# FudanCVL/SynFMC

Measured on AMD Instinct MI355X. Metric: denoising steps/sec, 16x320x512 bf16 U-Net+CMC+OMC, higher is better.
Workload: dtype bf16; 1 GPU; 16x320x512 clip, CFG batch 2, full-width 3D U-Net (1.39B params, random init) + Camera Adapter (CMC) + Object Motion Control (OMC) features, DDIM step; configs/obj.yaml shapes; 1 clip per GPU; frames=16, height=320, width=512, hip_graph=True, fp8_temporal_attention=False, parallelism=dp1 (independent clips, no collective)

## Files before the change

### include/fmc_hip.h

```cpp
#ifndef FMC_HIP_H
#define FMC_HIP_H

#include <stdint.h>

#ifdef __cplusplus
extern "C" {
#endif

#define FMC_VERSION 100

enum { FMC_BF16 = 0, FMC_F32 = 1 };

enum {
    FMC_OK = 0,
    FMC_E_SHAPE = -1,
    FMC_E_DTYPE = -2,
    FMC_E_ALIGN = -3,
    FMC_E_LAUNCH = -4,
    FMC_E_NULL = -5
};

int fmc_version(void);
const char* fmc_last_error(void);

int64_t fmc_groupnorm_workspace_bytes(int N, int C, int G);
int fmc_groupnorm_silu_fwd(const void* x, void* y, const float* gamma, const float* beta, float* stats,
                           void* workspace, int N, int HW, int C, int G, float eps, int act, int dtype,
                           const void* x2, int C1, void* stream);
int fmc_groupnorm_silu_bwd(const void* dy, const void* x, void* dx, const float* gamma, const float* beta,
                           const float* stats, void* workspace, int N, int HW, int C, int G, int act,
                           int dtype, void* stream);

int fmc_layernorm_fwd(const void* x, void* y, const float* gamma, const float* beta, const float* pe,
                      int64_t M, int C, float eps, int pe_inner, int pe_frames, int dtype, void* stream);
int fmc_layernorm_add_fwd(const void* x, const void* addend, void* sum_out, void* y, const float* gamma, const float* beta,
                          const float* pe, int64_t M, int C, float eps, int pe_inner, int pe_frames, int dtype, void* stream);

int fmc_geglu_fwd(const void* x, void* y, int64_t M, int Cff, int dtype, void* stream);

int fmc_spatial_attn_fwd(const void* q, const void* k, const void* v, void* o, float* lse, int B, int H,
                         int Sq, int Skv, int D, int64_t q_batch_stride, int64_t q_row_stride,
                         int64_t kv_batch_stride, int64_t kv_row_stride, int64_t o_batch_stride,
                         int64_t o_row_stride, int kv_batch_div, float scale, int dtype, void* stream);

int fmc_temporal_attn_fwd(const void* q, const void* k, const void* v, void* o, int n_clips, int n_pix,
                          int F, int H, int D, int64_t clip_stride, int64_t frame_stride,
                          int64_t pix_stride, int64_t o_clip_stride, int64_t o_frame_stride,
                          int64_t o_pix_stride, float scale, int dtype, void* stream);

int fmc_plucker_fwd(const float* K, const float* c2w, void* out, int B, int F, int H, int W, int c2w_rows,
                    int layout, int dtype, void* stream);

int fmc_omc_rasterize_fwd(const float* poses, const float* masks, void* feat, float* mask_out, int BF,
                          int n_obj, int H, int W, int layout, int dtype, void* stream);

int fmc_gaussian_circle_mask_fwd(const float* circles, float* out, int N, int H, int W, void* stream);

int fmc_mask_modulate_fwd(const void* x, const float* mask_in, void* y, float* mask_out, int N, int h, int w,
                          int C, int Hin, int Win, int dtype, void* stream);

int fmc_feature_add_fwd(const void* h, const void* t, void* out, int64_t n_elems, int64_t skip_elems,
                        int dtype, void* stream);

int fmc_cfg_ddim_step(const void* eps_uc, const float* x, float* x_out, int64_t n, int has_uncond,
                      float guidance, float alpha_t, float alpha_prev, int dtype, void* stream);

int fmc_linear_bf16(const void* x, const void* w, const void* bias, const void* residual, void* out, int64_t M, int N,
                    int K, int64_t ldx, int64_t ldres, int64_t ldo, float alpha, int epilogue, int tile, int split_k,
                    void* workspace, int64_t workspace_bytes, const void* x2, int64_t ldx2, int k_split,
                    const void* residual2, void* stream);

int fmc_conv3x3_bf16(const void* x, const void* w, const void* bias, const void* temb, const void* residual, void* out,
                     int n_img, int H, int W, int Cin, int Cout, int64_t temb_row_stride, int temb_img_div,
                     int upsample2x, int tile, int split_k, void* workspace, int64_t workspace_bytes, void* stream);

int fmc_linear_bf16_gn(const void* x, const void* w, const void* bias, const void* residual, void* out, int64_t M, int N, int K,
                       int64_t ldx, int64_t ldres, int64_t ldo, float alpha, const void* residual2, float* gn_partials, int gn_hw,
                       int w_tilemajor, void* stream);
int fmc_linear_bf16_ln(const void* x, const void* w, const void* bias, const void* residual, void* out, int64_t M, int N, int K,
                       int64_t ldx, int64_t ldres, int64_t ldo, float alpha, const void* residual2, void* ln_out, const float* ln_gamma,
                       const float* ln_beta, float ln_eps, const float* ln_pe, int ln_pe_inner, int ln_pe_frames, float* ln_stats, int w_tilemajor,
                       void* stream);
int fmc_linear_bf16_lnc(const void* x, const void* w_gamma, void* out, int64_t M, int N, int K, int64_t ldx, int64_t ldo, int epilogue,
                        const float* ln_stats, const float* ln_c, const float* ln_bias, int w_tilemajor, void* stream);
int fmc_linear_bf16_ffblk(const void* x, const void* w, const void* bias, const void* residual, void* out, int64_t M, int N, int K,
                          int64_t ldres, float alpha, int epilogue, int x_blocked, int out_blocked, const float* ln_stats, const float* ln_c,
                          const float* ln_bias, int w_tilemajor, void* stream);
int fmc_groupnorm_fold_linear(const float* partials, int part_splits, const float* gamma, const float* beta, const void* w, const void* bias,
                              void* w_out, float* bias_out, int n_img, int HW, int C, int G, int N, float eps, int w_tilemajor, void* stream);
int fmc_linear_bf16_imgw(const void* x, const void* w_img, const float* bias_img, void* out, int64_t M, int N, int K, int64_t ldx, int64_t ldo,
                         int img_rows, float* ln_stats, float ln_eps, int w_tilemajor, void* stream);
int fmc_linear_bf16_fftail(const void* x_blocked, const void* x2, const void* w, const void* bias, const void* residual, void* out, int64_t M,
                           int N, int K, int k_split, int64_t ldx2, int64_t ldres, float* gn_partials, int gn_hw, int w_tilemajor, void* stream);
int fmc_conv3x3_bf16_gn(const void* x, const void* w, const void* bias, const void* temb, const void* residual, void* out, int n_img,
                        int H, int W, int Cin, int Cout, int64_t temb_row_stride, int temb_img_div, int upsample2x,
                        float* gn_partials, int w_tilemajor, void* stream);
int fmc_groupnorm_apply_fwd(const void* x, void* y, const float* gamma, const float* beta, float* stats, const float* partials,
                            int part_splits, int N, int HW, int C, int G, float eps, int act, int dtype, void* stream);

int fmc_linear4_supported(int64_t M, int N, int K, int64_t ldx);
int fmc_linear4_bf16(const void* x, const void* w, const void* bias, const void* residual, const void* residual2, void* out, int64_t M, int N, int K,
                     int64_t ldx, int64_t ldres, int64_t ldo, float alpha, void* stream);

int fmc_vendor_init(void);
int fmc_vendor_destroy(void);
int fmc_vendor_version(void);
int64_t fmc_vendor_workspace_bytes(void);
int fmc_vendor_linear_candidates(int64_t M, int N, int K, int64_t ldx, int64_t ldres, int64_t ldo, int has_bias, int has_residual);
int fmc_vendor_linear_bf16(const void* x, const void* w, const void* bias, const void* residual, void* out, int64_t M, int N, int K,
                           int64_t ldx, int64_t ldres, int64_t ldo, int algo, void* workspace, int64_t workspace_bytes, void* stream);

int fmc_attention_supported(int D);
int fmc_attention_fwd(const void* q, const void* k, const void* v, void* o, const unsigned char* key_keep, int B, int H, int Sq, int Skv, int D,
                      int64_t q_batch_stride, int64_t q_row_stride, int64_t kv_batch_stride, int64_t kv_row_stride, int64_t o_batch_stride,
                      int64_t o_row_stride, float scale, int causal, int dtype, void* stream);

int fmc_geglu_pipe_supported(int64_t M, int cff, int C, int variant);
int fmc_geglu_pipe_ln_bf16(const void* h, void* out, const float* ln_gamma, const float* ln_beta, float ln_eps, const void* w_packed, const void* bias,
                           int64_t M, int cff, int C, int out_blocked, int variant, void* stream);

int fmc_groupnorm_partial_splits(int HW, int C);
int fmc_groupnorm_partials(const void* x, const void* x2, int C1, float* partials, int N, int HW, int C, int G, int dtype, void* stream);
int fmc_conv3x3_halo_supported(int n_img, int H, int W, int Cin, int Cin1, int Cout, int upsample2x);
int64_t fmc_conv3x3_halo_packed_bytes(int Cin, int Cout);
int fmc_conv3x3_halo_pack_weight(const void* w, void* dst, int Cin, int Cout, void* stream);
int fmc_conv3x3_halo_tiles_per_image(int H, int W);
int fmc_conv3x3_halo_bf16(const void* x, const void* x2, int Cin1, const void* w_packed, const void* bias, const void* temb, const void* residual,
                          void* out, int n_img, int H, int W, int Cin, int Cout, int64_t temb_row_stride, int temb_img_div, int upsample2x,
                          const float* gn_coef, int gn_act, float* gn_partials, void* stream);
int fmc_conv3x3_halo4_supported(int n_img, int H, int W, int Cin, int Cin1, int Cout, int upsample2x, int wide);
int fmc_conv3x3_halo4_pack_weight(const void* w, void* dst, int Cin, int Cout, int wide, void* stream);
int fmc_conv3x3_halo4_row_blocks_per_image(int H, int W);
int fmc_conv3x3_halo4_tiles(int n_img, int H, int W, int Cout, int wide);
int fmc_conv3x3_halo4_bf16(const void* x, const void* x2, int Cin1, const void* w_packed, const void* bias, const void* temb, const void* residual,
                           void* out, int n_img, int H, int W, int Cin, int Cout, int64_t temb_row_stride, int temb_img_div, int upsample2x,
                           float* gn_partials, int split_k, void* workspace, int64_t workspace_bytes, int wide, void* stream);
int fmc_groupnorm_coef(const float* partials, int part_splits, const float* gamma, const float* beta, float* coef, float* stats, int N, int HW,
                       int C, int G, float eps, void* stream);

int fmc_split_bf16x3(const float* src, void* dst, int64_t rows, int C, int64_t ld_src, int64_t ld_dst, int col0, int K,
                     int role, void* stream);
int fmc_linear_x3_f32(const void* x3, const void* w3, const float* bias, const float* residual, float* out, int64_t M, int N,
                      int K3, int64_t ldx, int64_t ldres, int64_t ldo, float alpha, int epilogue, int tile, int split_k,
                      void* workspace, int64_t workspace_bytes, const float* residual2, void* stream);
int fmc_conv3x3_x3_f32(const void* x3, const void* w3, const float* bias, const float* temb, const float* residual, float* out,
                       int n_img, int H, int W, int Cin3, int Cout, int64_t temb_row_stride, int temb_img_div,
                       int upsample2x, int tile, int split_k, void* workspace, int64_t workspace_bytes, void* stream);

int fmc_layernorm_bwd(const void* dy, const void* x, const float* gamma, void* dx, float* dgamma, float* dbeta,
                      int64_t M, int C, float eps, int dtype, void* stream);
int fmc_layernorm_bwd_add(const void* dy, const void* x, const float* gamma, void* dx, float* dgamma, float* dbeta, const void* addend,
                          int64_t M, int C, float eps, int dtype, void* stream);
int fmc_groupnorm_silu_bwd_add(const void* dy, const void* x, void* dx, const float* gamma, const float* beta, const float* stats,
                               void* workspace, int N, int HW, int C, int G, int act, const void* addend, int dtype, void* stream);
int64_t fmc_groupnorm_silu_bwd_params_workspace_bytes(int N, int HW, int C, int G);
int fmc_groupnorm_silu_bwd_params(const void* dy, const void* x, void* dx, float* dgamma, float* dbeta, const float* gamma,
                                  const float* beta, const float* stats, const void* addend, int accumulate, void* workspace,
                                  int N, int HW, int C, int G, int act, int dtype, void* stream);
int64_t fmc_column_sum_workspace_bytes(int64_t M, int N);
int fmc_column_sum(const void* x, float* out, int64_t M, int N, int64_t ld, float alpha, int accumulate, void* workspace, int dtype,
                   void* stream);
int fmc_geglu_bwd(const void* dy, const void* x, void* dx, int64_t M, int Cff, int dtype, void* stream);
int fmc_spatial_attn_bwd(const void* q, const void* k, const void* v, const void* o, const void* d_o, const float* lse,
                         float* dvec, void* dq, void* dk, void* dv, int B, int H, int Sq, int Skv, int D,
                         int64_t q_batch_stride, int64_t q_row_stride, int64_t kv_batch_stride, int64_t kv_row_stride,
                         int64_t o_batch_stride, int64_t o_row_stride, int64_t dq_batch_stride, int64_t dq_row_stride,
                         int64_t dkv_batch_stride, int64_t dkv_row_stride, int kv_batch_div, float scale, int dtype,
                         void* stream);
int fmc_temporal_attn_bwd(const void* q, const void* k, const void* v, const void* d_o, void* dq, void* dk, void* dv,
                          int n_clips, int n_pix, int F, int H, int D, int64_t clip_stride, int64_t frame_stride,
                          int64_t pix_stride, int64_t do_clip_stride, int64_t do_frame_stride, int64_t do_pix_stride,
                          int64_t dq_clip_stride, int64_t dq_frame_stride, int64_t dq_pix_stride, float scale,
                          int dtype, void* stream);

int fmc_fp8_scales_roll(void* amax, void* scale, void* inv_scale, float margin, void* stream);
int fmc_linear_fp8_qkv(const void* x, const void* w, void* out_fp8, int64_t M, int N, int K, int64_t ldx,
                       const void* inv_scales, void* amax_bits, void* stream);
int fmc_temporal_attn_fp8_fwd(const void* q, const void* k, const void* v, void* o, const void* scales, int n_clips,
                              int n_pix, int F, int H, int D, int64_t clip_stride, int64_t frame_stride,
                              int64_t pix_stride, int64_t o_clip_stride, int64_t o_frame_stride, int64_t o_pix_stride,
                              float scale, void* stream);
int fmc_temporal_attn_fp8_bwd(const void* q, const void* k, const void* v, const void* scales, const void* d_o, void* dq,
                              void* dk, void* dv, int n_clips, int n_pix, int F, int H, int D, int64_t clip_stride,
                              int64_t frame_stride, int64_t pix_stride, int64_t do_clip_stride, int64_t do_frame_stride,
                              int64_t do_pix_stride, int64_t dq_clip_stride, int64_t dq_frame_stride,
                              int64_t dq_pix_stride, float scale, void* stream);

int fmc_nhwc_to_cmajor_padded(const void* src, void* dst, int n_img, int H, int W, int C, int64_t row_len, int guard,
                              int shifts, void* stream);

typedef struct fmc_wgrad_problem {
    const void* a;
    const void* b;
    float* out;
    int64_t M, lda, ldb, ldo;
    int N, K;
    float alpha;
    int accumulate;
} fmc_wgrad_problem;
int64_t fmc_linear_wgrad_workspace_bytes(const fmc_wgrad_problem* problems, int n_problems);
int fmc_linear_wgrad_bf16(const fmc_wgrad_problem* problems, int n_problems, void* workspace, int64_t workspace_bytes, void* stream);

int fmc_temporal_block_bf16(const void* h, void* out, const float* ln_gamma, const float* ln_bpe, float ln_eps, const void* w_merge_tm,
                            const void* pose_term, float merge_scale, const void* w_qkv_packed, const void* w_out_tm, const void* b_out,
                            float* ln_stats, float ln_stats_eps, int n_clips, int frames, int hw, int channels, int heads, float scale,
                            void* stream);
int fmc_xattn_block640_bf16(const void* h, void* out, const float* ln_gamma, const float* ln_bpe, float ln_eps, const void* w_q_packed,
                            const void* kvfrag, const void* w_out_frag, const void* b_out, int n_images, int hw, int n_keys, int images_per_text,
                            float scale, void* stream);
int fmc_xattn_pack_kv(const void* kv, void* out, int batch, int S, int64_t ld_batch, void* stream);
int fmc_xattn_block320_bf16(const void* h, void* out, const float* ln_gamma, const float* ln_bpe, float ln_eps, const void* w_q_packed,
                            const void* kvfrag, const void* w_out_tm, const void* b_out, float* ln_stats, float ln_stats_eps, int n_images, int hw,
                            int n_keys, int images_per_text, float scale, void* stream);
int fmc_xattn_pack_kv40(const void* kv, void* out, int batch, int S, int64_t ld_batch, void* stream);
int fmc_geglu640_ln_bf16(const void* h, void* out, const float* ln_gamma, const float* ln_beta, float ln_eps, const void* w_packed, const void* bias,
                         int64_t M, int cff, int out_blocked, void* stream);
int fmc_geglu320_ln_bf16(const void* h, void* out, const float* ln_gamma, const float* ln_beta, float ln_eps, const void* w_packed, const void* bias,
                         int64_t M, int cff, int out_blocked, void* stream);
int fmc_temporal_block_set_debug(void* buf);

#ifdef __cplusplus
}
#endif
#endif
```

### synfmc_amd/_lib.py

```python
from __future__ import annotations

import ctypes
import os
from ctypes import c_char_p, c_float, c_int, c_int64, c_void_p

_HERE = os.path.dirname(os.path.abspath(__file__))
LIB_PATH = os.environ.get("FMC_HIP_LIB") or os.path.join(_HERE, "lib", "libfmc_hip.so")

FMC_BF16, FMC_F32 = 0, 1

_ERRORS = {-1: ValueError, -2: TypeError, -3: ValueError, -4: RuntimeError, -5: ValueError}

SIGNATURES = {
    "fmc_version": (c_int, []),
    "fmc_last_error": (c_char_p, []),
    "fmc_groupnorm_workspace_bytes": (c_int64, [c_int, c_int, c_int]),
    "fmc_groupnorm_silu_fwd": (c_int, [c_void_p, c_void_p, c_void_p, c_void_p, c_void_p, c_void_p, c_int, c_int, c_int,
                                       c_int, c_float, c_int, c_int, c_void_p, c_int, c_void_p]),
    "fmc_groupnorm_silu_bwd": (c_int, [c_void_p, c_void_p, c_void_p, c_void_p, c_void_p, c_void_p, c_void_p, c_int,
                                       c_int, c_int, c_int, c_int, c_int, c_void_p]),
    "fmc_layernorm_add_fwd": (c_int, [c_void_p, c_void_p, c_void_p, c_void_p, c_void_p, c_void_p, c_void_p, c_int64, c_int, c_float, c_int,
                                      c_int, c_int, c_void_p]),
    "fmc_layernorm_fwd": (c_int, [c_void_p, c_void_p, c_void_p, c_void_p, c_void_p, c_int64, c_int, c_float, c_int,
                                  c_int, c_int, c_void_p]),
    "fmc_geglu_fwd": (c_int, [c_void_p, c_void_p, c_int64, c_int, c_int, c_void_p]),
    "fmc_spatial_attn_fwd": (c_int, [c_void_p, c_void_p, c_void_p, c_void_p, c_void_p, c_int, c_int, c_int, c_int, c_int,
                                     c_int64, c_int64, c_int64, c_int64, c_int64, c_int64, c_int, c_float, c_int,
                                     c_void_p]),
    "fmc_temporal_attn_fwd": (c_int, [c_void_p, c_void_p, c_void_p, c_void_p, c_int, c_int, c_int, c_int, c_int,
                                      c_int64, c_int64, c_int64, c_int64, c_int64, c_int64, c_float, c_int, c_void_p]),
    "fmc_plucker_fwd": (c_int, [c_void_p, c_void_p, c_void_p, c_int, c_int, c_int, c_int, c_int, c_int, c_int, c_void_p]),
    "fmc_omc_rasterize_fwd": (c_int, [c_void_p, c_void_p, c_void_p, c_void_p, c_int, c_int, c_int, c_int, c_int, c_int,
                                      c_void_p]),
    "fmc_gaussian_circle_mask_fwd": (c_int, [c_void_p, c_void_p, c_int, c_int, c_int, c_void_p]),
    "fmc_mask_modulate_fwd": (c_int, [c_void_p, c_void_p, c_void_p, c_void_p, c_int, c_int, c_int, c_int, c_int, c_int,
                                      c_int, c_void_p]),
    "fmc_feature_add_fwd": (c_int, [c_void_p, c_void_p, c_void_p, c_int64, c_int64, c_int, c_void_p]),
    "fmc_cfg_ddim_step": (c_int, [c_void_p, c_void_p, c_void_p, c_int64, c_int, c_float, c_float, c_float, c_int,
                                  c_void_p]),
    "fmc_linear_bf16": (c_int, [c_void_p, c_void_p, c_void_p, c_void_p, c_void_p, c_int64, c_int, c_int, c_int64,
                                c_int64, c_int64, c_float, c_int, c_int, c_int, c_void_p, c_int64, c_void_p, c_int64, c_int,
                                c_void_p, c_void_p]),
    "fmc_linear_bf16_gn": (c_int, [c_void_p, c_void_p, c_void_p, c_void_p, c_void_p, c_int64, c_int, c_int, c_int64, c_int64, c_int64,
                                   c_float, c_void_p, c_void_p, c_int, c_int, c_void_p]),
    "fmc_linear_bf16_ln": (c_int, [c_void_p, c_void_p, c_void_p, c_void_p, c_void_p, c_int64, c_int, c_int, c_int64, c_int64, c_int64,
                                   c_float, c_void_p, c_void_p, c_void_p, c_void_p, c_float, c_void_p, c_int, c_int, c_void_p, c_int, c_void_p]),
    "fmc_linear_bf16_lnc": (c_int, [c_void_p, c_void_p, c_void_p, c_int64, c_int, c_int, c_int64, c_int64, c_int, c_void_p, c_void_p, c_void_p,
                                    c_int, c_void_p]),
    "fmc_linear_bf16_ffblk": (c_int, [c_void_p, c_void_p, c_void_p, c_void_p, c_void_p, c_int64, c_int, c_int, c_int64, c_float, c_int, c_int, c_int,
                                      c_void_p, c_void_p, c_void_p, c_int, c_void_p]),
    "fmc_groupnorm_fold_linear": (c_int, [c_void_p, c_int, c_void_p, c_void_p, c_void_p, c_void_p, c_void_p, c_void_p, c_int, c_int, c_int, c_int, c_int,
                                          c_float, c_int, c_void_p]),
    "fmc_linear_bf16_imgw": (c_int, [c_void_p, c_void_p, c_void_p, c_void_p, c_int64, c_int, c_int, c_int64, c_int64, c_int, c_void_p, c_float, c_int,
                                     c_void_p]),
    "fmc_linear_bf16_fftail": (c_int, [c_void_p, c_void_p, c_void_p, c_void_p, c_void_p, c_void_p, c_int64, c_int, c_int, c_int, c_int64, c_int64,
                                       c_void_p, c_int, c_int, c_void_p]),
    "fmc_conv3x3_bf16_gn": (c_int, [c_void_p, c_void_p, c_void_p, c_void_p, c_void_p, c_void_p, c_int, c_int, c_int, c_int, c_int,
                                    c_int64, c_int, c_int, c_void_p, c_int, c_void_p]),
    "fmc_groupnorm_partial_splits": (c_int, [c_int, c_int]),
    "fmc_groupnorm_partials": (c_int, [c_void_p, c_void_p, c_int, c_void_p, c_int, c_int, c_int, c_int, c_int, c_void_p]),
    "fmc_conv3x3_halo_supported": (c_int, [c_int, c_int, c_int, c_int, c_int, c_int, c_int]),
    "fmc_conv3x3_halo_packed_bytes": (c_int64, [c_int, c_int]),
    "fmc_conv3x3_halo_pack_weight": (c_int, [c_void_p, c_void_p, c_int, c_int, c_void_p]),
    "fmc_conv3x3_halo_tiles_per_image": (c_int, [c_int, c_int]),
    "fmc_conv3x3_halo_bf16": (c_int, [c_void_p, c_void_p, c_int, c_void_p, c_void_p, c_void_p, c_void_p, c_void_p, c_int, c_int, c_int, c_int, c_int,
                                      c_int64, c_int, c_int, c_void_p, c_int, c_void_p, c_void_p]),
    "fmc_conv3x3_halo4_supported": (c_int, [c_int, c_int, c_int, c_int, c_int, c_int, c_int, c_int]),
    "fmc_conv3x3_halo4_pack_weight": (c_int, [c_void_p, c_void_p, c_int, c_int, c_int, c_void_p]),
    "fmc_conv3x3_halo4_row_blocks_per_image": (c_int, [c_int, c_int]),
    "fmc_conv3x3_halo4_tiles": (c_int, [c_int, c_int, c_int, c_int, c_int]),
    "fmc_conv3x3_halo4_bf16": (c_int, [c_void_p, c_void_p, c_int, c_void_p, c_void_p, c_void_p, c_void_p, c_void_p, c_int, c_int, c_int, c_int, c_int,
                                       c_int64, c_int, c_int, c_void_p, c_int, c_void_p, c_int64, c_int, c_void_p]),
    "fmc_linear4_supported": (c_int, [c_int64, c_int, c_int, c_int64]),
    "fmc_vendor_linear_candidates": (c_int, [c_int64, c_int, c_int, c_int64, c_int64, c_int64, c_int, c_int]),
    "fmc_vendor_linear_bf16": (c_int, [c_void_p, c_void_p, c_void_p, c_void_p, c_void_p, c_int64, c_int, c_int, c_int64, c_int64, c_int64, c_int, c_void_p,
                                       c_int64, c_void_p]),
    "fmc_geglu_pipe_supported": (c_int, [c_int64, c_int, c_int, c_int]),
    "fmc_geglu_pipe_ln_bf16": (c_int, [c_void_p, c_void_p, c_void_p, c_void_p, c_float, c_void_p, c_void_p, c_int64, c_int, c_int, c_int, c_int, c_void_p]),
    "fmc_attention_supported": (c_int, [c_int]),
    "fmc_attention_fwd": (c_int, [c_void_p, c_void_p, c_void_p, c_void_p, c_void_p, c_int, c_int, c_int, c_int, c_int, c_int64, c_int64, c_int64, c_int64,
                                  c_int64, c_int64, c_float, c_int, c_int, c_void_p]),
    "fmc_vendor_init": (c_int, []),
    "fmc_vendor_destroy": (c_int, []),
    "fmc_vendor_version": (c_int, []),
    "fmc_vendor_workspace_bytes": (c_int64, []),
    "fmc_linear4_bf16": (c_int, [c_void_p, c_void_p, c_void_p, c_void_p, c_void_p, c_void_p, c_int64, c_int, c_int, c_int64, c_int64, c_int64, c_float, c_void_p]),
    "fmc_groupnorm_coef": (c_int, [c_void_p, c_int, c_void_p, c_void_p, c_void_p, c_void_p, c_int, c_int, c_int, c_int, c_float, c_void_p]),
    "fmc_groupnorm_apply_fwd": (c_int, [c_void_p, c_void_p, c_void_p, c_void_p, c_void_p, c_void_p, c_int, c_int, c_int, c_int, c_int,
                                        c_float, c_int, c_int, c_void_p]),
    "fmc_split_bf16x3": (c_int, [c_void_p, c_void_p, c_int64, c_int, c_int64, c_int64, c_int, c_int, c_int, c_void_p]),
    "fmc_linear_x3_f32": (c_int, [c_void_p, c_void_p, c_void_p, c_void_p, c_void_p, c_int64, c_int, c_int, c_int64,
                                  c_int64, c_int64, c_float, c_int, c_int, c_int, c_void_p, c_int64, c_void_p, c_void_p]),
    "fmc_conv3x3_x3_f32": (c_int, [c_void_p, c_void_p, c_void_p, c_void_p, c_void_p, c_void_p, c_int, c_int, c_int,
                                   c_int, c_int, c_int64, c_int, c_int, c_int, c_int, c_void_p, c_int64, c_void_p]),
    "fmc_layernorm_bwd": (c_int, [c_void_p, c_void_p, c_void_p, c_void_p, c_void_p, c_void_p, c_int64, c_int, c_float,
                                  c_int, c_void_p]),
    "fmc_layernorm_bwd_add": (c_int, [c_void_p, c_void_p, c_void_p, c_void_p, c_void_p, c_void_p, c_void_p, c_int64, c_int, c_float,
                                      c_int, c_void_p]),
    "fmc_groupnorm_silu_bwd_add": (c_int, [c_void_p, c_void_p, c_void_p, c_void_p, c_void_p, c_void_p, c_void_p, c_int, c_int, c_int, c_int,
                                           c_int, c_void_p, c_int, c_void_p]),
    "fmc_groupnorm_silu_bwd_params_workspace_bytes": (c_int64, [c_int, c_int, c_int, c_int]),
    "fmc_groupnorm_silu_bwd_params": (c_int, [c_void_p] * 9 + [c_int, c_void_p] + [c_int] * 6 + [c_void_p]),
    "fmc_column_sum_workspace_bytes": (c_int64, [c_int64, c_int]),
    "fmc_column_sum": (c_int, [c_void_p, c_void_p, c_int64, c_int, c_int64, c_float, c_int, c_void_p, c_int, c_void_p]),
    "fmc_geglu_bwd": (c_int, [c_void_p, c_void_p, c_void_p, c_int64, c_int, c_int, c_void_p]),
    "fmc_spatial_attn_bwd": (c_int, [c_void_p] * 10 + [c_int] * 5 + [c_int64] * 10 + [c_int, c_float, c_int, c_void_p]),
    "fmc_temporal_attn_bwd": (c_int, [c_void_p] * 7 + [c_int] * 5 + [c_int64] * 9 + [c_float, c_int, c_void_p]),
    "fmc_fp8_scales_roll": (c_int, [c_void_p, c_void_p, c_void_p, c_float, c_void_p]),
    "fmc_linear_fp8_qkv": (c_int, [c_void_p, c_void_p, c_void_p, c_int64, c_int, c_int, c_int64, c_void_p, c_void_p, c_void_p]),
    "fmc_temporal_attn_fp8_fwd": (c_int, [c_void_p] * 5 + [c_int] * 5 + [c_int64] * 6 + [c_float, c_void_p]),
    "fmc_temporal_attn_fp8_bwd": (c_int, [c_void_p] * 8 + [c_int] * 5 + [c_int64] * 9 + [c_float, c_void_p]),
    "fmc_nhwc_to_cmajor_padded": (c_int, [c_void_p, c_void_p, c_int, c_int, c_int, c_int, c_int64, c_int, c_int, c_void_p]),
    "fmc_linear_wgrad_workspace_bytes": (c_int64, [c_void_p, c_int]),
    "fmc_linear_wgrad_bf16": (c_int, [c_void_p, c_int, c_void_p, c_int64, c_void_p]),
    "fmc_temporal_block_bf16": (c_int, [c_void_p, c_void_p, c_void_p, c_void_p, c_float, c_void_p, c_void_p, c_float, c_void_p, c_void_p, c_void_p,
                                        c_void_p, c_float, c_int, c_int, c_int, c_int, c_int, c_float, c_void_p]),
    "fmc_temporal_block_set_debug": (c_int, [c_void_p]),
    "fmc_xattn_block640_bf16": (c_int, [c_void_p, c_void_p, c_void_p, c_void_p, c_float, c_void_p, c_void_p, c_void_p, c_void_p, c_int, c_int, c_int, c_int,
                                        c_float, c_void_p]),
    "fmc_xattn_pack_kv": (c_int, [c_void_p, c_void_p, c_int, c_int, c_int64, c_void_p]),
    "fmc_geglu320_ln_bf16": (c_int, [c_void_p, c_void_p, c_void_p, c_void_p, c_float, c_void_p, c_void_p, c_int64, c_int, c_int, c_void_p]),
    "fmc_geglu640_ln_bf16": (c_int, [c_void_p, c_void_p, c_void_p, c_void_p, c_float, c_void_p, c_void_p, c_int64, c_int, c_int, c_void_p]),
    "fmc_xattn_pack_kv40": (c_int, [c_void_p, c_void_p, c_int, c_int, c_int64, c_void_p]),
    "fmc_xattn_block320_bf16": (c_int, [c_void_p, c_void_p, c_void_p, c_void_p, c_float, c_void_p, c_void_p, c_void_p, c_void_p, c_void_p, c_float,
                                        c_int, c_int, c_int, c_int, c_float, c_void_p]),
    "fmc_conv3x3_bf16": (c_int, [c_void_p, c_void_p, c_void_p, c_void_p, c_void_p, c_void_p, c_int, c_int, c_int,
                                 c_int, c_int, c_int64, c_int, c_int, c_int, c_int, c_void_p, c_int64, c_void_p]),
}

_lib = None


class FmcLibraryMissing(ImportError):
    pass


def load() -> ctypes.CDLL:
    global _lib
    if _lib is not None:
        return _lib
    if not os.path.isfile(LIB_PATH):
        raise FmcLibraryMissing(
            f"{LIB_PATH} not found: build it with `make -C synfmc_amd/csrc` (hipcc --offload-arch=gfx950). "
            "There is no fallback path.")
    import torch
    lib = ctypes.CDLL(LIB_PATH)
    for name, (res, args) in SIGNATURES.items():
        fn = getattr(lib, name)
        fn.restype, fn.argtypes = res, args
    _lib = lib
    return lib


def check(rc: int, what: str) -> None:
    if rc != 0:
        msg = load().fmc_last_error()
        raise _ERRORS.get(rc, RuntimeError)(f"{what} failed ({rc}): {msg.decode() if msg else '?'}")
```

### synfmc_amd/csrc/conv_halo.hip

```cpp
#include <type_traits>

#include "common.h"

namespace {

constexpr int TH = 10, TW = 32, BM = TH * TW, BN = 160;
constexpr int HWID = TW + 2, HPIX = (TH + 2) * HWID;
constexpr int NP = 416;
constexpr int PLANE = NP * 16;
constexpr int HALO = 8 * PLANE;
constexpr int NBW = 5;
constexpr int WSUB = BN * 64;
constexpr int OFF_W = 2 * HALO, OFF_COEF = OFF_W + NBW * WSUB;
constexpr int LDS_BYTES = OFF_COEF + 2 * 512;
constexpr int NPIECE = 7;
constexpr unsigned OOB = 0x80000000u;

struct CHParams {
    const bf16_t* x; const bf16_t* x2;
    int c1;
    const bf16_t* w;
    const bf16_t* bias; const bf16_t* temb; const bf16_t* res; bf16_t* out;
    int n_img, H, W, cin, cout, ups;
    int64_t temb_ld; int temb_div;
    const float* gn_coef; int gn_act;
    float* gn_part;
    int tiles_y, tiles_x, tiles_n;
    int64_t x_bytes, x2_bytes, w_bytes;
};

template <int I> using IC = std::integral_constant<int, I>;

__device__ __forceinline__ float silu_fast(float z) { return z * __builtin_amdgcn_rcpf(1.f + __builtin_amdgcn_exp2f(-1.4426950408889634f * z)); }

constexpr int nh(int i) { return (i >= 0 && i <= 12 && (i & 1) == 0) ? 1 : 0; }

template <int GN>
__global__ __launch_bounds__(512, 2)
void conv_halo_kernel(const CHParams P) {
    extern __shared__ __attribute__((aligned(16))) unsigned char smem_raw[];
    const int tid = threadIdx.x, lane = tid & 63;
    const int wave = __builtin_amdgcn_readfirstlane(tid >> 6);
    const int half = wave >> 2, wq = wave & 3;
    const int wc = wq & 1, wr = half * 2 + (wq >> 1);
    const int l15 = lane & 15, kq = lane >> 4;
    const bool clsA = wave < 2;

    int tile_p, tile_n;
    {
        const int total = P.n_img * P.tiles_y * P.tiles_x * P.tiles_n;
        const int id = blockIdx.x, q = total >> 3, r = total & 7, xcd = id & 7;
        const int lin = (xcd < r ? xcd * (q + 1) : r * (q + 1) + (xcd - r) * q) + (id >> 3);
        tile_p = lin / P.tiles_n;
        tile_n = lin - tile_p * P.tiles_n;
    }
    const int tpi = P.tiles_y * P.tiles_x;
    const int img = tile_p / tpi, tin = tile_p - img * tpi;
    const int y0 = (tin / P.tiles_x) * TH, x0 = (tin % P.tiles_x) * TW;
    const int n0 = tile_n * BN;
    const int nchunk = P.cin >> 6, nsub = nchunk * 18;

    const int Hs = P.ups ? P.H >> 1 : P.H, Ws = P.ups ? P.W >> 1 : P.W;
    const int pp = lane & 7, pg = ((lane & 7) + (lane >> 3)) & 7;
    int h_pix[NPIECE];
#pragma unroll
    for (int j = 0; j < NPIECE; ++j) {
        const int b = 8 * j + wave, px = 8 * b + pp;
        const int hy = px / HWID, hx = px - hy * HWID;
        const int y = y0 - 1 + hy, x = x0 - 1 + hx;
        const bool in = b < HPIX / 8 && (unsigned)y < (unsigned)P.H && (unsigned)x < (unsigned)P.W;
        const int ys = P.ups ? y >> 1 : y, xs = P.ups ? x >> 1 : x;
        h_pix[j] = in ? (img * Hs + ys) * Ws + xs : -1;
    }
    const int h_lds = pg * PLANE + (8 * wave + pp) * 16;
    const bool last_piece = wave < HPIX / 8 - 48;
    const __amdgpu_buffer_rsrc_t rsX = __builtin_amdgcn_make_buffer_rsrc((void*)P.x, 0, (int)P.x_bytes, 0x00020000);
    const __amdgpu_buffer_rsrc_t rsX2 = __builtin_amdgcn_make_buffer_rsrc((void*)(P.x2 ? P.x2 : P.x), 0, (int)(P.x2 ? P.x2_bytes : P.x_bytes), 0x00020000);
    const __amdgpu_buffer_rsrc_t rsW = __builtin_amdgcn_make_buffer_rsrc((void*)P.w, 0, (int)P.w_bytes, 0x00020000);
    const int c2 = P.cin - P.c1;
    u32x4 hreg[2];
    auto halo_load = [&](int j, int ch64, u32x4& dst) {
        const int cbeg = ch64 * 64;
        const bool second = cbeg >= P.c1, past = ch64 >= nchunk;
        const int pitch = past ? 0 : (second ? c2 : P.c1) * 2;
        const unsigned coff = past ? OOB : (unsigned)(((second ? cbeg - P.c1 : cbeg) + pg * 8) * 2);
        unsigned vo = (unsigned)(h_pix[j] * pitch) + coff;
        vo = h_pix[j] < 0 ? OOB : vo;
        const __amdgpu_buffer_rsrc_t rs = second ? rsX2 : rsX;
        dst = __builtin_bit_cast(u32x4, __builtin_amdgcn_raw_buffer_load_b128(rs, (int)vo, 0, 0));
    };
    auto halo_transform = [&](int j, int coefbuf, const u32x4& raw) -> u32x4 {
        if constexpr (GN == 0) return raw;
        const f32x4* src = reinterpret_cast<const f32x4*>(smem_raw + OFF_COEF + coefbuf * 512 + pg * 64);
        float f[8];
#pragma unroll
        for (int k = 0; k < 4; ++k) { f[2 * k] = __uint_as_float(raw[k] << 16); f[2 * k + 1] = __uint_as_float(raw[k] & 0xffff0000u); }
#pragma unroll
        for (int k = 0; k < 4; ++k) {
            const f32x4 t = src[k];
            const float z0 = fmaf(f[2 * k], t[0], t[1]), z1 = fmaf(f[2 * k + 1], t[2], t[3]);
            f[2 * k] = GN == 1 ? silu_fast(z0) : z0;
            f[2 * k + 1] = GN == 1 ? silu_fast(z1) : z1;
        }
        const bool in = h_pix[j] >= 0;
        u32x4 v;
#pragma unroll
        for (int k = 0; k < 4; ++k) v[k] = in ? pack_bf2(f[2 * k], f[2 * k + 1]) : 0u;
        return v;
    };
    auto halo_store = [&](int j, int buf, const u32x4& v) {
        if (j == NPIECE - 1 && !last_piece) return;
        *reinterpret_cast<u32x4*>(smem_raw + buf * HALO + h_lds + j * 1024) = v;
    };
    auto coef_fetch = [&](int ch64) -> float {
        const int cc = ch64 < nchunk ? ch64 : nchunk - 1;
        const float* src = GN ? P.gn_coef + ((size_t)img * P.cin + cc * 64) * 2 + (tid & 127) : reinterpret_cast<const float*>(P.w);
        return *src;
    };

    const int my_piece = clsA ? 2 * wave : wave + 2;
    const unsigned w_vo0 = (unsigned)(lane * 16 + my_piece * 1024);
    const int w_dst0 = OFF_W + my_piece * 1024;
    int iss_soff = tile_n * nsub * WSUB, iss_left = nsub, iss_slot = 0;
    auto w_issue = [&](auto cls) {
        unsigned char* dst = smem_raw + w_dst0 + iss_slot * WSUB;
        __builtin_amdgcn_raw_ptr_buffer_load_lds(rsW, (__attribute__((address_space(3))) void*)dst, 16, (int)w_vo0, iss_soff, 0, 0);
        if constexpr (decltype(cls)::value)
            __builtin_amdgcn_raw_ptr_buffer_load_lds(rsW, (__attribute__((address_space(3))) void*)(dst + 1024), 16, (int)w_vo0, iss_soff + 1024, 0, 0);
        iss_soff += WSUB;
        if (--iss_left == 0) { iss_left = nsub; iss_soff = tile_n * nsub * WSUB; }
        iss_slot = iss_slot + 1 == NBW ? 0 : iss_slot + 1;
    };

    f32x4 acc[5][5];
    bf16x8 wf[5], af[5];
    const int wfrag = OFF_W + ((wc * 80 + l15) * 32 + (kq ^ (3 * ((l15 >> 3) & 1))) * 8) * 2;
    int afrag[5];
#pragma unroll
    for (int mb = 0; mb < 5; ++mb) {
        const int idx = wr * 80 + mb * 16 + l15, ty = idx >> 5, tx = idx & 31;
        afrag[mb] = kq * PLANE + (ty * HWID + tx) * 16;
    }

    {
        u32x4 t[NPIECE];
#pragma unroll
        for (int j = 0; j < NPIECE; ++j) halo_load(j, 0, t[j]);
        const float c0v = coef_fetch(0), c1v = coef_fetch(1);
        if (tid < 128) {
            *reinterpret_cast<float*>(smem_raw + OFF_COEF + tid * 4) = c0v;
            *reinterpret_cast<float*>(smem_raw + OFF_COEF + 512 + tid * 4) = c1v;
        }
        __syncthreads();
#pragma unroll
        for (int j = 0; j < NPIECE; ++j) halo_store(j, 0, halo_transform(j, 0, t[j]));
    }
    asm volatile("s_waitcnt vmcnt(0) lgkmcnt(0)" ::: "memory");

    auto main_loop = [&](auto cls) {
        constexpr int NW = decltype(cls)::value ? 2 : 1;
        int rd_slot = 0;
        w_issue(cls); w_issue(cls); w_issue(cls);
        asm volatile("s_waitcnt vmcnt(%0)" ::"n"(2 * NW) : "memory");
        __builtin_amdgcn_s_barrier();
        if (half == 1) __builtin_amdgcn_s_barrier();
        __builtin_amdgcn_sched_barrier(0);
#pragma unroll
        for (int a = 0; a < 5; ++a)
#pragma unroll
            for (int b = 0; b < 5; ++b) acc[a][b] = f32x4{0.f, 0.f, 0.f, 0.f};
        __builtin_amdgcn_sched_barrier(0);

        int cbuf = 0;
        float coef_next = 0.f;
        u32x4 hpk = {0u, 0u, 0u, 0u};
        for (int c = 0; c < nchunk; ++c) {
            const int abase = cbuf * HALO, nbuf = cbuf ^ 1;
            auto sub = [&](auto ic) {
                constexpr int i = decltype(ic)::value;
                constexpr int tap = i >> 1, hk = i & 1, ky = tap / 3, kx = tap % 3;
                constexpr int aimm = hk * 4 * PLANE + (ky * HWID + kx) * 16;
                if constexpr (i >= 3 && i <= 15 && (i & 1) == 1) halo_store((i - 3) / 2, nbuf, hpk);
                if constexpr (i == 16) {
                    if (tid < 128) *reinterpret_cast<float*>(smem_raw + OFF_COEF + cbuf * 512 + tid * 4) = coef_next;
                }
                {
                    const unsigned char* Wp = smem_raw + wfrag + rd_slot * WSUB;
#pragma unroll
                    for (int nb = 0; nb < 5; ++nb) wf[nb] = __builtin_bit_cast(bf16x8, *reinterpret_cast<const u32x4*>(Wp + nb * 1024));
#pragma unroll
                    for (int mb = 0; mb < 5; ++mb)
                        af[mb] = __builtin_bit_cast(bf16x8, *reinterpret_cast<const u32x4*>(smem_raw + abase + afrag[mb] + aimm));
                    rd_slot = rd_slot + 1 == NBW ? 0 : rd_slot + 1;
                }
                if constexpr (nh(i) == 1) halo_load(i / 2, c + 1, hreg[(i / 2) & 1]);
                if constexpr (i == 13) coef_next = coef_fetch(c + 2);
                w_issue(cls);
                {
                    constexpr int extra = nh(i - 1) + nh(i) + (i == 13 || i == 14 ? 1 : 0);
                    asm volatile("s_waitcnt vmcnt(%0)" ::"n"(2 * NW + extra) : "memory");
                }
                __builtin_amdgcn_sched_barrier(0);
                __builtin_amdgcn_s_barrier();
                __builtin_amdgcn_sched_barrier(0);
                __builtin_amdgcn_s_setprio(1);
                if constexpr (i >= 2 && i <= 14 && (i & 1) == 0) hpk = halo_transform((i - 2) / 2, nbuf, hreg[((i - 2) / 2) & 1]);
#pragma unroll
                for (int mb = 0; mb < 5; ++mb)
#pragma unroll
                    for (int nb = 0; nb < 5; ++nb)
                        acc[mb][nb] = __builtin_amdgcn_mfma_f32_16x16x32_bf16(wf[nb], af[mb], acc[mb][nb], 0, 0, 0);
                if constexpr (GN != 0 && i >= 2 && i <= 14 && (i & 1) == 0) {
#pragma unroll
                    for (int k = 0; k < 25; ++k) {
                        __builtin_amdgcn_sched_group_barrier(0x008, 1, 0);
                        __builtin_amdgcn_sched_group_barrier(0x102, 3, 0);
                    }
                }
                __builtin_amdgcn_s_setprio(0);
                __builtin_amdgcn_sched_barrier(0);
                __builtin_amdgcn_s_barrier();
                __builtin_amdgcn_sched_barrier(0);
            };
            sub(IC<0>{}); sub(IC<1>{}); sub(IC<2>{}); sub(IC<3>{}); sub(IC<4>{}); sub(IC<5>{});
            sub(IC<6>{}); sub(IC<7>{}); sub(IC<8>{}); sub(IC<9>{}); sub(IC<10>{}); sub(IC<11>{});
            sub(IC<12>{}); sub(IC<13>{}); sub(IC<14>{}); sub(IC<15>{}); sub(IC<16>{}); sub(IC<17>{});
            cbuf = nbuf;
        }
    };
    if (clsA) main_loop(std::true_type{}); else main_loop(std::false_type{});
    if (half == 0) __builtin_amdgcn_s_barrier();
    asm volatile("s_waitcnt vmcnt(0)" ::: "memory");
    __syncthreads();

    constexpr int OP = BN + 8;
    bf16_t* Os = reinterpret_cast<bf16_t*>(smem_raw);
    constexpr int CPR = BN / 8;
    const int vrows = min(TH, P.H - y0) * TW;
    auto row_pixel = [&](int r) -> int64_t { return ((int64_t)img * P.H + y0 + (r >> 5)) * P.W + x0 + (r & 31); };
    {
        u32x2 bt[5], tt[5];
        if (P.bias) {
#pragma unroll
            for (int nb = 0; nb < 5; ++nb) bt[nb] = *reinterpret_cast<const u32x2*>(P.bias + n0 + wc * 80 + nb * 16 + 4 * kq);
        }
        if (P.temb) {
            const bf16_t* trow = P.temb + (int64_t)(img / P.temb_div) * P.temb_ld + n0 + wc * 80 + 4 * kq;
#pragma unroll
            for (int nb = 0; nb < 5; ++nb) tt[nb] = *reinterpret_cast<const u32x2*>(trow + nb * 16);
        }
#pragma unroll
        for (int nb = 0; nb < 5; ++nb) {
            float b4[4] = {0.f, 0.f, 0.f, 0.f};
            if (P.bias) {
                b4[0] = __uint_as_float(bt[nb][0] << 16); b4[1] = __uint_as_float(bt[nb][0] & 0xffff0000u);
                b4[2] = __uint_as_float(bt[nb][1] << 16); b4[3] = __uint_as_float(bt[nb][1] & 0xffff0000u);
            }
            if (P.temb) {
                b4[0] += __uint_as_float(tt[nb][0] << 16); b4[1] += __uint_as_float(tt[nb][0] & 0xffff0000u);
                b4[2] += __uint_as_float(tt[nb][1] << 16); b4[3] += __uint_as_float(tt[nb][1] & 0xffff0000u);
            }
#pragma unroll
            for (int mb = 0; mb < 5; ++mb)
#pragma unroll
                for (int j = 0; j < 4; ++j) acc[mb][nb][j] += b4[j];
        }
    }
    if (P.res) {
#pragma unroll
        for (int h = 0; h < 2; ++h) {
            u32x4 rv[7];
#pragma unroll
            for (int it = 0; it < 7; ++it) {
                const int cidx = min(tid + (7 * h + it) * 512, BM * CPR - 1), r = cidx / CPR, ch = cidx - r * CPR;
                rv[it] = *reinterpret_cast<const u32x4*>(P.res + row_pixel(r < vrows ? r : 0) * P.cout + n0 + ch * 8);
            }
#pragma unroll
            for (int it = 0; it < 7; ++it) {
                const int cidx = tid + (7 * h + it) * 512, r = cidx / CPR, ch = cidx - r * CPR;
                if (cidx < BM * CPR) *reinterpret_cast<u32x4*>(Os + r * OP + ch * 8) = rv[it];
            }
        }
        __syncthreads();
#pragma unroll
        for (int mb = 0; mb < 5; ++mb)
#pragma unroll
            for (int nb = 0; nb < 5; ++nb) {
                const u32x2 t = *reinterpret_cast<const u32x2*>(Os + (wr * 80 + mb * 16 + l15) * OP + wc * 80 + nb * 16 + 4 * kq);
                acc[mb][nb][0] += __uint_as_float(t[0] << 16); acc[mb][nb][1] += __uint_as_float(t[0] & 0xffff0000u);
                acc[mb][nb][2] += __uint_as_float(t[1] << 16); acc[mb][nb][3] += __uint_as_float(t[1] & 0xffff0000u);
            }
        __syncthreads();
    }
#pragma unroll
    for (int mb = 0; mb < 5; ++mb)
#pragma unroll
        for (int nb = 0; nb < 5; ++nb)
            *reinterpret_cast<u32x2*>(Os + (wr * 80 + mb * 16 + l15) * OP + wc * 80 + nb * 16 + 4 * kq) =
                u32x2{pack_bf2(acc[mb][nb][0], acc[mb][nb][1]), pack_bf2(acc[mb][nb][2], acc[mb][nb][3])};
    __syncthreads();
    float gs = 0.f, gss = 0.f;
    const int cpg = P.cout >> 5, GT = BN / cpg, RP = 512 / GT;
    if (P.gn_part) {
        const int gl = tid % GT;
        for (int r = tid / GT; r < vrows; r += RP) {
            const unsigned* wsrc = reinterpret_cast<const unsigned*>(Os + r * OP + gl * cpg);
            for (int k = 0; k < cpg / 2; ++k) {
                const unsigned u = wsrc[k];
                const float a = __uint_as_float(u << 16), b = __uint_as_float(u & 0xffff0000u);
                gs += a + b;
                gss += a * a + b * b;
            }
        }
    }
    for (int cidx = tid; cidx < BM * CPR; cidx += 512) {
        const int r = cidx / CPR, ch = cidx - r * CPR;
        if (r < vrows)
            *reinterpret_cast<u32x4*>(P.out + row_pixel(r) * P.cout + n0 + ch * 8) = *reinterpret_cast<const u32x4*>(Os + r * OP + ch * 8);
    }
    if (P.gn_part) {
        float* red = reinterpret_cast<float*>(smem_raw + (size_t)BM * OP * 2);
        red[2 * tid] = gs;
        red[2 * tid + 1] = gss;
        __syncthreads();
        if (tid < GT) {
            float a = 0.f, b = 0.f;
            for (int k = 0; k < RP; ++k) { a += red[2 * (tid + k * GT)]; b += red[2 * (tid + k * GT) + 1]; }
            float* dst = P.gn_part + (((int64_t)img * tpi + tin) * 32 + (n0 / cpg + tid)) * 2;
            dst[0] = a;
            dst[1] = b;
        }
    }
}

__global__ __launch_bounds__(256) void conv_halo_pack_kernel(const bf16_t* __restrict__ w, bf16_t* __restrict__ dst, int cout, int cin) {
    const int64_t total = (int64_t)cout * 9 * cin / 8;
    for (int64_t id = (int64_t)blockIdx.x * blockDim.x + threadIdx.x; id < total; id += (int64_t)gridDim.x * blockDim.x) {
        int64_t t = id;
        const int p = (int)(t & 3); t >>= 2;
        const int row = (int)(t % BN); t /= BN;
        const int hk = (int)(t & 1); t >>= 1;
        const int tap = (int)(t % 9); t /= 9;
        const int nchunk = cin >> 6;
        const int ch64 = (int)(t % nchunk); t /= nchunk;
        const int nt = (int)t;
        const int lc = p ^ (3 * ((row >> 3) & 1));
        const int64_t src = (((int64_t)(nt * BN + row) * 9 + tap) * cin + ch64 * 64 + hk * 32 + lc * 8);
        *reinterpret_cast<u32x4*>(dst + id * 8) = *reinterpret_cast<const u32x4*>(w + src);
    }
}

__global__ __launch_bounds__(256) void gn_coef_kernel(const float* __restrict__ part, int splits, const float* __restrict__ gamma,
                                                      const float* __restrict__ beta, float* __restrict__ coef, float* __restrict__ stats,
                                                      int C, int G, double count, float eps) {
    __shared__ float s_mean[64], s_rstd[64];
    const int n = blockIdx.x;
    if ((int)threadIdx.x < G) {
        double a = 0.0, b = 0.0;
        for (int s = 0; s < splits; ++s) {
            const float* p = part + (((int64_t)n * splits + s) * G + threadIdx.x) * 2;
            a += (double)p[0];
            b += (double)p[1];
        }
        const double mean = a / count;
        double var = b / count - mean * mean;
        if (var < 0.0) var = 0.0;
        const float rstd = (float)(1.0 / sqrt(var + (double)eps));
        s_mean[threadIdx.x] = (float)mean;
        s_rstd[threadIdx.x] = rstd;
        if (stats) { stats[((int64_t)n * G + threadIdx.x) * 2] = (float)mean; stats[((int64_t)n * G + threadIdx.x) * 2 + 1] = rstd; }
    }
    __syncthreads();
    const int cpg = C / G;
    for (int c = threadIdx.x; c < C; c += blockDim.x) {
        const int g = c / cpg;
        const float a = s_rstd[g] * gamma[c];
        coef[((int64_t)n * C + c) * 2] = a;
        coef[((int64_t)n * C + c) * 2 + 1] = beta[c] - s_mean[g] * a;
    }
}

}

extern "C" int64_t fmc_conv3x3_halo_packed_bytes(int Cin, int Cout) { return (int64_t)Cout * 9 * Cin * 2; }

extern "C" int fmc_conv3x3_halo_pack_weight(const void* w, void* dst, int Cin, int Cout, void* stream) {
    if (!w || !dst) FMC_FAIL(FMC_E_NULL, "conv3x3_halo_pack_weight: NULL pointer");
    if (Cin % 64 || Cout % BN) FMC_FAIL(FMC_E_SHAPE, "conv3x3_halo_pack_weight: Cin %% 64 / Cout %% 160 (Cin=%d Cout=%d)", Cin, Cout);
    if (!fmc_aligned16(w) || !fmc_aligned16(dst)) FMC_FAIL(FMC_E_ALIGN, "conv3x3_halo_pack_weight: pointers must be 16-byte aligned");
    const int64_t chunks = (int64_t)Cout * 9 * Cin / 8;
    const int grid = (int)((chunks + 255) / 256 < 4096 ? (chunks + 255) / 256 : 4096);
    hipLaunchKernelGGL(conv_halo_pack_kernel, dim3(grid), dim3(256), 0, (hipStream_t)stream, (const bf16_t*)w, (bf16_t*)dst, Cout, Cin);
    FMC_CHECK_LAUNCH("fmc_conv3x3_halo_pack_weight");
    return 0;
}

extern "C" int fmc_conv3x3_halo_supported(int n_img, int H, int W, int Cin, int Cin1, int Cout, int upsample2x) {
    if (n_img < 1 || H < 1 || W < 1 || W % TW || Cin % 64 || Cout % BN) return 0;
    if (Cin1 <= 0 || Cin1 > Cin || Cin1 % 64) return 0;
    if (upsample2x && ((H | W) & 1)) return 0;
    const int64_t hs = upsample2x ? H / 2 : H, ws = upsample2x ? W / 2 : W;
    if ((int64_t)n_img * hs * ws * Cin1 * 2 >= (1ll << 31) || (int64_t)n_img * hs * ws * (Cin - Cin1) * 2 >= (1ll << 31)) return 0;
    if ((int64_t)Cout * 9 * Cin * 2 >= (1ll << 31)) return 0;
    return 1;
}

extern "C" int fmc_conv3x3_halo_bf16(const void* x, const void* x2, int Cin1, const void* w_packed, const void* bias, const void* temb,
                                     const void* residual, void* out, int n_img, int H, int W, int Cin, int Cout, int64_t temb_row_stride,
                                     int temb_img_div, int upsample2x, const float* gn_coef, int gn_act, float* gn_partials, void* stream) {
    if (!x || !w_packed || !out) FMC_FAIL(FMC_E_NULL, "conv3x3_halo: NULL x / w / out");
    if (!x2) Cin1 = Cin;
    if (!fmc_conv3x3_halo_supported(n_img, H, W, Cin, Cin1, Cout, upsample2x))
        FMC_FAIL(FMC_E_SHAPE, "conv3x3_halo: needs W %% 32 == 0, Cin %% 64 == 0 (both sources), Cout %% 160 == 0, operands < 2 GiB "
                 "(n=%d H=%d W=%d Cin=%d+%d Cout=%d ups=%d)", n_img, H, W, Cin1, Cin - Cin1, Cout, upsample2x);
    if (!fmc_aligned16(x) || !fmc_aligned16(w_packed) || !fmc_aligned16(out) || (x2 && !fmc_aligned16(x2)) || (residual && !fmc_aligned16(residual)) ||
        (bias && (reinterpret_cast<uintptr_t>(bias) & 7)) || (temb && ((reinterpret_cast<uintptr_t>(temb) & 7) || temb_row_stride % 4)))
        FMC_FAIL(FMC_E_ALIGN, "conv3x3_halo: x / w / out / residual must be 16-byte aligned, bias / temb rows 8-byte aligned");
    if (temb && temb_img_div < 1) FMC_FAIL(FMC_E_SHAPE, "conv3x3_halo: temb_img_div %d", temb_img_div);
    if (gn_partials && (Cout % 64 || BN % (Cout / 32)))
        FMC_FAIL(FMC_E_SHAPE, "conv3x3_halo: the statistics epilogue needs Cout %% 64 == 0 and 160 %% (Cout / 32) == 0 (Cout=%d)", Cout);
    CHParams P;
    P.x = (const bf16_t*)x; P.x2 = (const bf16_t*)x2; P.c1 = Cin1;
    P.w = (const bf16_t*)w_packed; P.bias = (const bf16_t*)bias; P.temb = (const bf16_t*)temb; P.res = (const bf16_t*)residual; P.out = (bf16_t*)out;
    P.n_img = n_img; P.H = H; P.W = W; P.cin = Cin; P.cout = Cout; P.ups = upsample2x ? 1 : 0;
    P.temb_ld = temb_row_stride; P.temb_div = temb ? temb_img_div : 1;
    P.gn_coef = gn_coef; P.gn_act = gn_act; P.gn_part = gn_partials;
    P.tiles_y = (H + TH - 1) / TH; P.tiles_x = W / TW; P.tiles_n = Cout / BN;
    const int64_t hs = upsample2x ? H / 2 : H, ws = upsample2x ? W / 2 : W;
    P.x_bytes = (int64_t)n_img * hs * ws * Cin1 * 2; P.x2_bytes = (int64_t)n_img * hs * ws * (Cin - Cin1) * 2;
    P.w_bytes = (int64_t)Cout * 9 * Cin * 2;
    static FmcPerDeviceFlag raised;
    if (!raised) {
        (void)hipFuncSetAttribute(reinterpret_cast<const void*>(&conv_halo_kernel<0>), hipFuncAttributeMaxDynamicSharedMemorySize, LDS_BYTES);
        (void)hipFuncSetAttribute(reinterpret_cast<const void*>(&conv_halo_kernel<1>), hipFuncAttributeMaxDynamicSharedMemorySize, LDS_BYTES);
        (void)hipFuncSetAttribute(reinterpret_cast<const void*>(&conv_halo_kernel<2>), hipFuncAttributeMaxDynamicSharedMemorySize, LDS_BYTES);
        raised = true;
    }
    const unsigned grid = (unsigned)(n_img * P.tiles_y * P.tiles_x * P.tiles_n);
    if (!gn_coef) hipLaunchKernelGGL(conv_halo_kernel<0>, dim3(grid), dim3(512), LDS_BYTES, (hipStream_t)stream, P);
    else if (gn_act) hipLaunchKernelGGL(conv_halo_kernel<1>, dim3(grid), dim3(512), LDS_BYTES, (hipStream_t)stream, P);
    else hipLaunchKernelGGL(conv_halo_kernel<2>, dim3(grid), dim3(512), LDS_BYTES, (hipStream_t)stream, P);
    FMC_CHECK_LAUNCH("fmc_conv3x3_halo_bf16");
    return 0;
}

extern "C" int fmc_conv3x3_halo_tiles_per_image(int H, int W) { return ((H + TH - 1) / TH) * (W / TW); }

extern "C" int fmc_groupnorm_coef(const float* partials, int part_splits, const float* gamma, const float* beta, float* coef, float* stats,
                                  int N, int HW, int C, int G, float eps, void* stream) {
    if (!partials || !gamma || !beta || !coef) FMC_FAIL(FMC_E_NULL, "groupnorm_coef: NULL pointer");
    if (N < 1 || C < 1 || G < 1 || G > 64 || C % G || part_splits < 1) FMC_FAIL(FMC_E_SHAPE, "groupnorm_coef: N=%d C=%d G=%d splits=%d", N, C, G, part_splits);
    hipLaunchKernelGGL(gn_coef_kernel, dim3((unsigned)N), dim3(256), 0, (hipStream_t)stream, partials, part_splits, gamma, beta, coef, stats, C, G,
                       (double)HW * (double)(C / G), eps);
    FMC_CHECK_LAUNCH("fmc_groupnorm_coef");
    return 0;
}
```

### synfmc_amd/csrc/conv_halo4.hip

```cpp
#include <type_traits>

#include "common.h"

namespace {

constexpr int BM = 320;
#ifndef FMC_C4_INTERLEAVE
#define FMC_C4_INTERLEAVE 1
#endif
constexpr bool INTERLEAVE = FMC_C4_INTERLEAVE != 0;
constexpr unsigned OOB = 0x80000000u;

template <int TW, int NWV> struct Geo {
    static constexpr int BN = 20 * NWV, NT = 64 * NWV;
    static constexpr int WSUB = BN * 64;
    static constexpr int WPIECES = BN / 16;
    static constexpr int TH = TW == 8 ? 5 : 10;
    static constexpr int RB = TH * TW;
    static constexpr int NB = BM / RB;
    static constexpr int HW_ = TW + 2, HB = (TH + 2) * HW_;
    static constexpr int HPIX = NB * HB;
    static constexpr int NP = (HPIX + 15) / 16 * 16;
    static constexpr int PLANE = NP * 16, HALO = 8 * PLANE;
    static constexpr int NBW = (2 * HALO + 5 * WSUB <= 163840) ? 5 : 4;
    static constexpr int DW = NBW - 1;
    static constexpr int OFF_W = 2 * HALO;
    static constexpr int LDS_BYTES = OFF_W + NBW * WSUB;
    static constexpr int NPIECE = (HPIX / 8 + NWV - 1) / NWV;
    static_assert(HPIX % 8 == 0 && LDS_BYTES <= 163840 && NPIECE <= 18, "geometry");
};

struct C4Params {
    const bf16_t* x; const bf16_t* x2; int c1;
    const bf16_t* w;
    const bf16_t* bias; const bf16_t* temb; const bf16_t* res; bf16_t* out;
    int n_img, H, W, cin, cout, ups;
    int64_t temb_ld; int temb_div;
    float* gn_part;
    int tiles_y, tiles_x, tiles_p, tiles_n;
    int splits; float* ws;
    int64_t x_bytes, x2_bytes, w_bytes;
    int xcd_pc;
};

template <int I> using IC = std::integral_constant<int, I>;

template <int NPIECE> constexpr int pps() { return NPIECE > 12 ? 2 : 1; }
template <int NPIECE> constexpr int nh(int i) {
    return (i >= 0 && pps<NPIECE>() * i < NPIECE) ? (pps<NPIECE>() == 2 && 2 * i + 1 < NPIECE ? 2 : 1) : 0;
}

template <int TW, int NWV>
__global__ __launch_bounds__(64 * NWV, NWV / 4)
void conv_halo4_kernel(const C4Params P) {
    using G = Geo<TW, NWV>;
    constexpr int BN = G::BN, NT = G::NT, WSUB = G::WSUB;
    constexpr int TH = G::TH, RB = G::RB, NB = G::NB, HW_ = G::HW_, HB = G::HB, PLANE = G::PLANE, HALO = G::HALO, NBW = G::NBW, OFF_W = G::OFF_W;
    constexpr int NPIECE = G::NPIECE, DW = G::DW;
    extern __shared__ __attribute__((aligned(16))) unsigned char smem_raw[];
    const int tid = threadIdx.x, lane = tid & 63;
    const int wave = __builtin_amdgcn_readfirstlane(tid >> 6);
    const int l15 = lane & 15, kq = lane >> 4;
    const int wp = wave & 3, wn = wave >> 2;
    const bool clsA = wave < G::WPIECES - NWV;

    int tile_p, tile_n, split;
    {
        const int total = P.tiles_p * P.tiles_n * P.splits;
        const int id = blockIdx.x, xcd = id & 7;
        if (P.xcd_pc > 0) {
            const int j = id >> 3, pc = P.xcd_pc;
            const int tnl = P.tiles_n * P.splits / pc, tpl = P.tiles_p / (8 / pc);
            const int tnv = (xcd % pc) * tnl + j % tnl;
            tile_p = (xcd / pc) * tpl + j / tnl;
            split = tnv % P.splits;
            tile_n = tnv / P.splits;
        } else {
            const int q = total >> 3, r = total & 7;
            int lin = (xcd < r ? xcd * (q + 1) : r * (q + 1) + (xcd - r) * q) + (id >> 3);
            split = lin % P.splits;
            lin /= P.splits;
            tile_p = lin / P.tiles_n;
            tile_n = lin - tile_p * P.tiles_n;
        }
    }
    const int n0 = tile_n * BN;
    const int nchunk_all = P.cin >> 6;
    const int per = (nchunk_all + P.splits - 1) / P.splits;
    const int ck0 = split * per, nchunk = max(0, min(nchunk_all, ck0 + per) - ck0);
    const int nsub = max(nchunk, 1) * 18;
    const int tpi = P.tiles_y * P.tiles_x;
    const int rb0 = tile_p * NB, rb_total = P.n_img * tpi;

    const int Hs = P.ups ? P.H >> 1 : P.H, Ws = P.ups ? P.W >> 1 : P.W;
    const int pp = lane & 7, pg = ((lane & 7) + (lane >> 3)) & 7;
    int h_pix[NPIECE];
#pragma unroll
    for (int j = 0; j < NPIECE; ++j) {
        const int b = NWV * j + wave, px = 8 * b + pp;
        const int blk = px / HB, rem = px - blk * HB;
        const int hy = rem / HW_, hx = rem - hy * HW_;
        const int rb = rb0 + blk;
        const int img = rb / tpi, rin = rb - img * tpi, yb = rin / P.tiles_x, xb = rin - yb * P.tiles_x;
        const int y = yb * TH - 1 + hy, x = xb * TW - 1 + hx;
        const bool in = px < G::HPIX && rb < rb_total && (unsigned)y < (unsigned)P.H && (unsigned)x < (unsigned)P.W;
        const int ys = P.ups ? y >> 1 : y, xs = P.ups ? x >> 1 : x;
        h_pix[j] = in ? (img * Hs + ys) * Ws + xs : -1;
    }
    const int h_lds = pg * PLANE + (8 * wave + pp) * 16;
    const __amdgpu_buffer_rsrc_t rsX = __builtin_amdgcn_make_buffer_rsrc((void*)P.x, 0, (int)P.x_bytes, 0x00020000);
    const __amdgpu_buffer_rsrc_t rsX2 = __builtin_amdgcn_make_buffer_rsrc((void*)(P.x2 ? P.x2 : P.x), 0, (int)(P.x2 ? P.x2_bytes : P.x_bytes), 0x00020000);
    const __amdgpu_buffer_rsrc_t rsW = __builtin_amdgcn_make_buffer_rsrc((void*)P.w, 0, (int)P.w_bytes, 0x00020000);
    const int c2 = P.cin - P.c1;
    auto halo_load = [&](int j, int crel) -> u32x4 {
        const int cbeg = (ck0 + crel) * 64;
        const bool second = cbeg >= P.c1, past = crel >= nchunk;
        const int pitch = past ? 0 : (second ? c2 : P.c1) * 2;
        const unsigned coff = past ? OOB : (unsigned)(((second ? cbeg - P.c1 : cbeg) + pg * 8) * 2);
        unsigned vo = (unsigned)(h_pix[j] * pitch) + coff;
        vo = h_pix[j] < 0 ? OOB : vo;
        const __amdgpu_buffer_rsrc_t rs = second ? rsX2 : rsX;
        return __builtin_bit_cast(u32x4, __builtin_amdgcn_raw_buffer_load_b128(rs, (int)vo, 0, 0));
    };
    auto halo_store = [&](int j, int buf, const u32x4& v) {
        if (8 * (NWV * j + wave) < G::HPIX)
            *reinterpret_cast<u32x4*>(smem_raw + buf * HALO + h_lds + j * (128 * NWV)) = v;
    };

    const unsigned w_vo0 = (unsigned)(lane * 16 + wave * 1024);
    const int w_base = (tile_n * nchunk_all + ck0) * 18 * WSUB;
    int iss_soff = w_base, iss_left = nsub, iss_slot = 0;
    auto w_issue = [&](auto cls) {
        unsigned char* dst = smem_raw + OFF_W + iss_slot * WSUB + wave * 1024;
        __builtin_amdgcn_raw_ptr_buffer_load_lds(rsW, (__attribute__((address_space(3))) void*)dst, 16, (int)w_vo0, iss_soff, 0, 0);
        if constexpr (decltype(cls)::value)
            __builtin_amdgcn_raw_ptr_buffer_load_lds(rsW, (__attribute__((address_space(3))) void*)(dst + NWV * 1024), 16, (int)w_vo0, iss_soff + NWV * 1024, 0, 0);
        iss_soff += WSUB;
        if (--iss_left == 0) { iss_left = nsub; iss_soff = w_base; }
        iss_slot = iss_slot + 1 == NBW ? 0 : iss_slot + 1;
    };

    f32x4 acc[5][5];
    bf16x8 wf[2][5], af[2][5];
    const int wfrag = OFF_W + ((wn * 80 + l15) * 32 + (kq ^ (3 * ((l15 >> 3) & 1))) * 8) * 2;
    int afrag[5];
#pragma unroll
    for (int mb = 0; mb < 5; ++mb) {
        const int idx = wp * 80 + mb * 16 + l15, blk = idx / RB, r = idx - blk * RB, ty = r / TW, tx = r - ty * TW;
        afrag[mb] = kq * PLANE + (blk * HB + ty * HW_ + tx) * 16;
    }

    {
        u32x4 t[NPIECE];
#pragma unroll
        for (int j = 0; j < NPIECE; ++j) t[j] = halo_load(j, 0);
#pragma unroll
        for (int j = 0; j < NPIECE; ++j) halo_store(j, 0, t[j]);
    }
    asm volatile("s_waitcnt vmcnt(0) lgkmcnt(0)" ::: "memory");

    auto main_loop = [&](auto cls) {
        constexpr int NW = decltype(cls)::value ? 2 : 1;
        constexpr int PPS = pps<NPIECE>();
        u32x4 hreg[3][PPS];
        w_issue(cls); w_issue(cls); w_issue(cls);
        if constexpr (DW == 4) w_issue(cls);
        asm volatile("s_waitcnt vmcnt(%0)" ::"n"((DW - 1) * NW) : "memory");
        __builtin_amdgcn_s_barrier();
        int rd_slot = 0;
        auto read_frags = [&](int set, int abase, int aimm) {
            const unsigned char* Wp = smem_raw + wfrag + rd_slot * WSUB;
#pragma unroll
            for (int nb = 0; nb < 5; ++nb) wf[set][nb] = __builtin_bit_cast(bf16x8, *reinterpret_cast<const u32x4*>(Wp + nb * 1024));
#pragma unroll
            for (int mb = 0; mb < 5; ++mb)
                af[set][mb] = __builtin_bit_cast(bf16x8, *reinterpret_cast<const u32x4*>(smem_raw + abase + afrag[mb] + aimm));
            rd_slot = rd_slot + 1 == NBW ? 0 : rd_slot + 1;
        };
        read_frags(0, 0, 0);
#pragma unroll
        for (int a = 0; a < 5; ++a)
#pragma unroll
            for (int b = 0; b < 5; ++b) acc[a][b] = f32x4{0.f, 0.f, 0.f, 0.f};

        int cbuf = 0;
        for (int c = 0; c < nchunk; ++c) {
            const int abase = cbuf * HALO, nbuf = cbuf ^ 1;
            auto sub = [&](auto ic) {
                constexpr int i = decltype(ic)::value;
                constexpr int n1 = (i + 1) % 18, tap1 = n1 >> 1, hk1 = n1 & 1;
                constexpr int aimm1 = hk1 * 4 * PLANE + ((tap1 / 3) * HW_ + (tap1 % 3)) * 16;
                {
                    constexpr int extra = nh<NPIECE>(i - 1) + (DW == 4 ? nh<NPIECE>(i - 2) : 0);
                    asm volatile("s_waitcnt vmcnt(%0)" ::"n"((DW - 2) * NW + extra) : "memory");
                }
                __builtin_amdgcn_sched_barrier(0);
                __builtin_amdgcn_s_barrier();
                __builtin_amdgcn_sched_barrier(0);
                if constexpr (nh<NPIECE>(i - 3) >= 1) halo_store(PPS * (i - 3), nbuf, hreg[(i - 3) % 3][0]);
                if constexpr (nh<NPIECE>(i - 3) == 2) halo_store(PPS * (i - 3) + 1, nbuf, hreg[(i - 3) % 3][PPS - 1]);
                read_frags((i + 1) & 1, i == 17 ? nbuf * HALO : abase, aimm1);
                if constexpr (nh<NPIECE>(i) >= 1) hreg[i % 3][0] = halo_load(PPS * i, c + 1);
                if constexpr (nh<NPIECE>(i) == 2) hreg[i % 3][PPS - 1] = halo_load(PPS * i + 1, c + 1);
                w_issue(cls);
#pragma unroll
                for (int mb = 0; mb < 5; ++mb)
#pragma unroll
                    for (int nb = 0; nb < 5; ++nb)
                        acc[mb][nb] = __builtin_amdgcn_mfma_f32_16x16x32_bf16(wf[i & 1][nb], af[i & 1][mb], acc[mb][nb], 0, 0, 0);
                if constexpr (INTERLEAVE) {
#pragma unroll
                    for (int k = 0; k < 2; ++k) {
                        __builtin_amdgcn_sched_group_barrier(0x008, 1, 0);
                        __builtin_amdgcn_sched_group_barrier(0x200, 1, 0);
                    }
#pragma unroll
                    for (int k = 0; k < 10; ++k) {
                        __builtin_amdgcn_sched_group_barrier(0x008, 1, 0);
                        __builtin_amdgcn_sched_group_barrier(0x100, 1, 0);
                    }
#pragma unroll
                    for (int k = 0; k < 4; ++k) {
                        __builtin_amdgcn_sched_group_barrier(0x008, 1, 0);
                        __builtin_amdgcn_sched_group_barrier(0x020, 1, 0);
                    }
                    __builtin_amdgcn_sched_group_barrier(0x008, 9, 0);
                }
                __builtin_amdgcn_sched_barrier(0);
            };
            sub(IC<0>{}); sub(IC<1>{}); sub(IC<2>{}); sub(IC<3>{}); sub(IC<4>{}); sub(IC<5>{});
            sub(IC<6>{}); sub(IC<7>{}); sub(IC<8>{}); sub(IC<9>{}); sub(IC<10>{}); sub(IC<11>{});
            sub(IC<12>{}); sub(IC<13>{}); sub(IC<14>{}); sub(IC<15>{}); sub(IC<16>{}); sub(IC<17>{});
            cbuf = nbuf;
        }
    };
    if (clsA) main_loop(std::true_type{}); else main_loop(std::false_type{});
    asm volatile("s_waitcnt vmcnt(0) lgkmcnt(0)" ::: "memory");
    __syncthreads();

    if (P.splits > 1) {
        const int64_t mtot = (int64_t)P.n_img * P.H * P.W;
#pragma unroll
        for (int mb = 0; mb < 5; ++mb) {
            const int r = wp * 80 + mb * 16 + l15;
            const int blk = r / RB, q = r - blk * RB, ty = q / TW, tx = q - ty * TW;
            const int rb = rb0 + blk, img = rb / tpi, rin = rb - img * tpi, yb = rin / P.tiles_x, xb = rin - yb * P.tiles_x, y = yb * TH + ty;
            if (rb < rb_total && y < P.H) {
                float* dst = P.ws + ((int64_t)split * mtot + ((int64_t)img * P.H + y) * P.W + xb * TW + tx) * P.cout + n0 + wn * 80 + 4 * kq;
#pragma unroll
                for (int nb = 0; nb < 5; ++nb) *reinterpret_cast<f32x4*>(dst + nb * 16) = acc[mb][nb];
            }
        }
        return;
    }
    constexpr int OP = BN + 8;
    bf16_t* Os = reinterpret_cast<bf16_t*>(smem_raw);
    constexpr int CPR = BN / 8;
    auto row_pixel = [&](int r, bool& ok) -> int64_t {
        const int blk = r / RB, q = r - blk * RB, ty = q / TW, tx = q - ty * TW;
        const int rb = rb0 + blk, img = rb / tpi, rin = rb - img * tpi, yb = rin / P.tiles_x, xb = rin - yb * P.tiles_x, y = yb * TH + ty;
        ok = rb < rb_total && y < P.H;
        return ((int64_t)img * P.H + y) * P.W + xb * TW + tx;
    };
    {
        u32x2 bt[5], tt[5][5];
        if (P.bias) {
#pragma unroll
            for (int nb = 0; nb < 5; ++nb) bt[nb] = *reinterpret_cast<const u32x2*>(P.bias + n0 + wn * 80 + nb * 16 + 4 * kq);
        }
        if (P.temb) {
#pragma unroll
            for (int mb = 0; mb < 5; ++mb) {
                const int idx = wp * 80 + mb * 16 + l15, rb = min(rb0 + idx / RB, rb_total - 1), img = rb / tpi;
                const bf16_t* trow = P.temb + (int64_t)(img / P.temb_div) * P.temb_ld + n0 + wn * 80 + 4 * kq;
#pragma unroll
                for (int nb = 0; nb < 5; ++nb) tt[mb][nb] = *reinterpret_cast<const u32x2*>(trow + nb * 16);
            }
        }
#pragma unroll
        for (int nb = 0; nb < 5; ++nb) {
            float b4[4] = {0.f, 0.f, 0.f, 0.f};
            if (P.bias) {
                b4[0] = __uint_as_float(bt[nb][0] << 16); b4[1] = __uint_as_float(bt[nb][0] & 0xffff0000u);
                b4[2] = __uint_as_float(bt[nb][1] << 16); b4[3] = __uint_as_float(bt[nb][1] & 0xffff0000u);
            }
#pragma unroll
            for (int mb = 0; mb < 5; ++mb) {
                float t4[4] = {0.f, 0.f, 0.f, 0.f};
                if (P.temb) {
                    t4[0] = __uint_as_float(tt[mb][nb][0] << 16); t4[1] = __uint_as_float(tt[mb][nb][0] & 0xffff0000u);
                    t4[2] = __uint_as_float(tt[mb][nb][1] << 16); t4[3] = __uint_as_float(tt[mb][nb][1] & 0xffff0000u);
                }
#pragma unroll
                for (int j = 0; j < 4; ++j) acc[mb][nb][j] += b4[j] + t4[j];
            }
        }
    }
    if (P.res) {
        constexpr int NIT = (BM * CPR + NT - 1) / NT, RBU = 7;
#pragma unroll
        for (int h = 0; h < (NIT + RBU - 1) / RBU; ++h) {
            u32x4 rv[RBU];
#pragma unroll
            for (int it = 0; it < RBU; ++it) {
                const int cidx = min(tid + (h * RBU + it) * NT, BM * CPR - 1), r = cidx / CPR, ch = cidx - r * CPR;
                bool ok;
                const int64_t m = row_pixel(r, ok);
                rv[it] = *reinterpret_cast<const u32x4*>(P.res + (ok ? m : 0) * P.cout + n0 + ch * 8);
            }
#pragma unroll
            for (int it = 0; it < RBU; ++it) {
                const int cidx = tid + (h * RBU + it) * NT, r = cidx / CPR, ch = cidx - r * CPR;
                if (cidx < BM * CPR) *reinterpret_cast<u32x4*>(Os + r * OP + ch * 8) = rv[it];
            }
        }
        __syncthreads();
#pragma unroll
        for (int mb = 0; mb < 5; ++mb)
#pragma unroll
            for (int nb = 0; nb < 5; ++nb) {
                const u32x2 t = *reinterpret_cast<const u32x2*>(Os + (wp * 80 + mb * 16 + l15) * OP + wn * 80 + nb * 16 + 4 * kq);
                acc[mb][nb][0] += __uint_as_float(t[0] << 16); acc[mb][nb][1] += __uint_as_float(t[0] & 0xffff0000u);
                acc[mb][nb][2] += __uint_as_float(t[1] << 16); acc[mb][nb][3] += __uint_as_float(t[1] & 0xffff0000u);
            }
        __syncthreads();
    }
#pragma unroll
    for (int mb = 0; mb < 5; ++mb)
#pragma unroll
        for (int nb = 0; nb < 5; ++nb)
            *reinterpret_cast<u32x2*>(Os + (wp * 80 + mb * 16 + l15) * OP + wn * 80 + nb * 16 + 4 * kq) =
                u32x2{pack_bf2(acc[mb][nb][0], acc[mb][nb][1]), pack_bf2(acc[mb][nb][2], acc[mb][nb][3])};
    __syncthreads();
    for (int cidx = tid; cidx < BM * CPR; cidx += NT) {
        const int r = cidx / CPR, ch = cidx - r * CPR;
        bool ok;
        const int64_t m = row_pixel(r, ok);
        if (ok) *reinterpret_cast<u32x4*>(P.out + m * P.cout + n0 + ch * 8) = *reinterpret_cast<const u32x4*>(Os + r * OP + ch * 8);
    }
    if (P.gn_part) {
        const int cpg = P.cout >> 5, GT = BN / cpg, RP = NT / GT, gl = tid % GT;
        float* red = reinterpret_cast<float*>(smem_raw + (size_t)BM * OP * 2);
        for (int blk = 0; blk < NB; ++blk) {
            const int rb = rb0 + blk;
            if (rb >= rb_total) break;
            const int img = rb / tpi, sp = rb - img * tpi;
            const int vr = min(TH, P.H - (sp / P.tiles_x) * TH) * TW;
            float gs = 0.f, gss = 0.f;
            for (int r = tid / GT; r < vr; r += RP) {
                const unsigned* wsrc = reinterpret_cast<const unsigned*>(Os + (blk * RB + r) * OP + gl * cpg);
                for (int k = 0; k < cpg / 2; ++k) {
                    const unsigned u = wsrc[k];
                    const float a = __uint_as_float(u << 16), b = __uint_as_float(u & 0xffff0000u);
                    gs += a + b;
                    gss += a * a + b * b;
                }
            }
            red[2 * tid] = gs;
            red[2 * tid + 1] = gss;
            __syncthreads();
            if (tid < GT) {
                float a = 0.f, b = 0.f;
                for (int k = 0; k < RP; ++k) { a += red[2 * (tid + k * GT)]; b += red[2 * (tid + k * GT) + 1]; }
                float* dst = P.gn_part + (((int64_t)img * tpi + sp) * 32 + (n0 / cpg + tid)) * 2;
                dst[0] = a;
                dst[1] = b;
            }
            __syncthreads();
        }
    }
}

__global__ __launch_bounds__(256) void conv_halo4_pack_kernel(const bf16_t* __restrict__ w, bf16_t* __restrict__ dst, int cout, int cin, int BN) {
    const int64_t total = (int64_t)cout * 9 * cin / 8;
    for (int64_t id = (int64_t)blockIdx.x * blockDim.x + threadIdx.x; id < total; id += (int64_t)gridDim.x * blockDim.x) {
        int64_t t = id;
        const int p = (int)(t & 3); t >>= 2;
        const int row = (int)(t % BN); t /= BN;
        const int hk = (int)(t & 1); t >>= 1;
        const int tap = (int)(t % 9); t /= 9;
        const int nchunk = cin >> 6;
        const int ch64 = (int)(t % nchunk); t /= nchunk;
        const int nt = (int)t;
        const int lc = p ^ (3 * ((row >> 3) & 1));
        const int64_t src = (((int64_t)(nt * BN + row) * 9 + tap) * cin + ch64 * 64 + hk * 32 + lc * 8);
        *reinterpret_cast<u32x4*>(dst + id * 8) = *reinterpret_cast<const u32x4*>(w + src);
    }
}

__global__ __launch_bounds__(256) void conv_halo4_finish_kernel(const C4Params P) {
    const int64_t mtot = (int64_t)P.n_img * P.H * P.W, cpr = P.cout / 8, total = mtot * cpr;
    for (int64_t id = (int64_t)blockIdx.x * blockDim.x + threadIdx.x; id < total; id += (int64_t)gridDim.x * blockDim.x) {
        const int64_t m = id / cpr;
        const int n = (int)(id - m * cpr) * 8;
        u32x4 tb = u32x4{0u, 0u, 0u, 0u}, tt = tb, tr = tb;
        if (P.bias) tb = *reinterpret_cast<const u32x4*>(P.bias + n);
        if (P.temb) tt = *reinterpret_cast<const u32x4*>(P.temb + ((m / ((int64_t)P.H * P.W)) / P.temb_div) * P.temb_ld + n);
        if (P.res) tr = *reinterpret_cast<const u32x4*>(P.res + m * P.cout + n);
        float v[8] = {0.f, 0.f, 0.f, 0.f, 0.f, 0.f, 0.f, 0.f};
        for (int sp0 = 0; sp0 < P.splits; sp0 += 4) {
            f32x4 pa[4], pb[4];
#pragma unroll
            for (int k = 0; k < 4; ++k) {
                const float* src = P.ws + ((int64_t)min(sp0 + k, P.splits - 1) * mtot + m) * P.cout + n;
                pa[k] = *reinterpret_cast<const f32x4*>(src);
                pb[k] = *reinterpret_cast<const f32x4*>(src + 4);
            }
#pragma unroll
            for (int k = 0; k < 4; ++k)
                if (sp0 + k < P.splits) {
#pragma unroll
                    for (int j = 0; j < 4; ++j) { v[j] += pa[k][j]; v[4 + j] += pb[k][j]; }
                }
        }
        const u32x4* side[3] = {&tb, &tt, &tr};
#pragma unroll
        for (int q = 0; q < 3; ++q)
#pragma unroll
            for (int j = 0; j < 4; ++j) {
                v[2 * j] += __uint_as_float((*side[q])[j] << 16);
                v[2 * j + 1] += __uint_as_float((*side[q])[j] & 0xffff0000u);
            }
        Vec8<bf16_t>::store(P.out + m * P.cout + n, v);
    }
}

template <int TW, int NWV> int launch_c4(C4Params& P, hipStream_t st) {
    using G = Geo<TW, NWV>;
    P.tiles_y = (P.H + G::TH - 1) / G::TH;
    P.tiles_x = P.W / TW;
    P.tiles_p = (P.n_img * P.tiles_y * P.tiles_x + G::NB - 1) / G::NB;
    {
        static const int forced = getenv("FMC_C4_XCD") ? atoi(getenv("FMC_C4_XCD")) : -1;
        const int tnv = P.tiles_n * P.splits;
        double best = 0.;
        P.xcd_pc = 0;
        if (forced != 0 && (P.tiles_p * tnv) % 8 == 0) {
            for (int pc = 1; pc <= 8; pc *= 2) {
                if (tnv % pc || P.tiles_p % (8 / pc) || (forced > 0 && pc != forced)) continue;
                const double cost = (double)P.w_bytes * (8 / pc) + (double)(P.x_bytes + P.x2_bytes) * pc;
                if (!P.xcd_pc || cost < best) { best = cost; P.xcd_pc = pc; }
            }
        }
    }
    static FmcPerDeviceFlag raised;
    if (!raised) {
        (void)hipFuncSetAttribute(reinterpret_cast<const void*>(&conv_halo4_kernel<TW, NWV>), hipFuncAttributeMaxDynamicSharedMemorySize, G::LDS_BYTES);
        raised = true;
    }
    hipLaunchKernelGGL((conv_halo4_kernel<TW, NWV>), dim3((unsigned)(P.tiles_p * P.tiles_n * P.splits)), dim3(G::NT), G::LDS_BYTES, st, P);
    if (P.splits > 1) {
        const int64_t chunks = (int64_t)P.n_img * P.H * P.W * (P.cout / 8);
        const unsigned grid = (unsigned)((chunks + 255) / 256 < 2048 ? (chunks + 255) / 256 : 2048);
        hipLaunchKernelGGL(conv_halo4_finish_kernel, dim3(grid), dim3(256), 0, st, P);
    }
    return 0;
}

}

extern "C" int fmc_conv3x3_halo4_pack_weight(const void* w, void* dst, int Cin, int Cout, int wide, void* stream) {
    const int BN = wide ? 160 : 80;
    if (!w || !dst) FMC_FAIL(FMC_E_NULL, "conv3x3_halo4_pack_weight: NULL pointer");
    if (Cin % 64 || Cout % BN) FMC_FAIL(FMC_E_SHAPE, "conv3x3_halo4_pack_weight: Cin %% 64 / Cout %% %d (Cin=%d Cout=%d)", BN, Cin, Cout);
    if (!fmc_aligned16(w) || !fmc_aligned16(dst)) FMC_FAIL(FMC_E_ALIGN, "conv3x3_halo4_pack_weight: pointers must be 16-byte aligned");
    const int64_t chunks = (int64_t)Cout * 9 * Cin / 8;
    const int grid = (int)((chunks + 255) / 256 < 4096 ? (chunks + 255) / 256 : 4096);
    hipLaunchKernelGGL(conv_halo4_pack_kernel, dim3(grid), dim3(256), 0, (hipStream_t)stream, (const bf16_t*)w, (bf16_t*)dst, Cout, Cin, BN);
    FMC_CHECK_LAUNCH("fmc_conv3x3_halo4_pack_weight");
    return 0;
}

static int c4_tw(int W) { return W % 16 == 0 ? 16 : 8; }
extern "C" int fmc_conv3x3_halo4_supported(int n_img, int H, int W, int Cin, int Cin1, int Cout, int upsample2x, int wide) {
    if (n_img < 1 || H < 1 || W < 8 || W % 8 || Cin % 64 || Cout % (wide ? 160 : 80) || (wide && W % 16)) return 0;
    if (Cin1 <= 0 || Cin1 > Cin || Cin1 % 64) return 0;
    if (upsample2x && ((H | W) & 1)) return 0;
    const int64_t hs = upsample2x ? H / 2 : H, ws = upsample2x ? W / 2 : W;
    if ((int64_t)n_img * hs * ws * Cin1 * 2 >= (1ll << 31) || (int64_t)n_img * hs * ws * (Cin - Cin1) * 2 >= (1ll << 31)) return 0;
    if ((int64_t)Cout * 9 * Cin * 2 >= (1ll << 31)) return 0;
    return 1;
}

extern "C" int fmc_conv3x3_halo4_row_blocks_per_image(int H, int W) {
    const int tw = c4_tw(W);
    return (tw == 8 ? (H + 4) / 5 : (H + 9) / 10) * (W / tw);
}

extern "C" int fmc_conv3x3_halo4_tiles(int n_img, int H, int W, int Cout, int wide) {
    const int nb = c4_tw(W) == 8 ? 8 : 2;
    return (n_img * fmc_conv3x3_halo4_row_blocks_per_image(H, W) + nb - 1) / nb * (Cout / (wide ? 160 : 80));
}

extern "C" int fmc_conv3x3_halo4_bf16(const void* x, const void* x2, int Cin1, const void* w_packed, const void* bias, const void* temb,
                                      const void* residual, void* out, int n_img, int H, int W, int Cin, int Cout, int64_t temb_row_stride,
                                      int temb_img_div, int upsample2x, float* gn_partials, int split_k, void* workspace, int64_t workspace_bytes,
                                      int wide, void* stream) {
    const int BN = wide ? 160 : 80;
    if (!x || !w_packed || !out) FMC_FAIL(FMC_E_NULL, "conv3x3_halo4: NULL x / w / out");
    if (!x2) Cin1 = Cin;
    if (!fmc_conv3x3_halo4_supported(n_img, H, W, Cin, Cin1, Cout, upsample2x, wide))
        FMC_FAIL(FMC_E_SHAPE, "conv3x3_halo4: needs W %% 8 == 0 (wide: %% 16), Cin %% 64 == 0 (both sources), Cout %% %d == 0, operands < 2 GiB "
                 "(n=%d H=%d W=%d Cin=%d+%d Cout=%d ups=%d)", BN, n_img, H, W, Cin1, Cin - Cin1, Cout, upsample2x);
    if (!fmc_aligned16(x) || !fmc_aligned16(w_packed) || !fmc_aligned16(out) || (x2 && !fmc_aligned16(x2)) || (residual && !fmc_aligned16(residual)) ||
        (bias && (reinterpret_cast<uintptr_t>(bias) & 7)) || (temb && ((reinterpret_cast<uintptr_t>(temb) & 7) || temb_row_stride % 4)))
        FMC_FAIL(FMC_E_ALIGN, "conv3x3_halo4: x / w / out / residual must be 16-byte aligned, bias / temb rows 8-byte aligned");
    if (temb && temb_img_div < 1) FMC_FAIL(FMC_E_SHAPE, "conv3x3_halo4: temb_img_div %d", temb_img_div);
    if (gn_partials && (Cout % 64 || BN % (Cout / 32)))
        FMC_FAIL(FMC_E_SHAPE, "conv3x3_halo4: the statistics epilogue needs Cout %% 64 == 0 and %d %% (Cout / 32) == 0 (Cout=%d)", BN, Cout);
    if (split_k < 1) split_k = 1;
    if (split_k > Cin / 64) split_k = Cin / 64;
    if (split_k > 1) {
        if (gn_partials) FMC_FAIL(FMC_E_SHAPE, "conv3x3_halo4: the statistics epilogue is not available with split_k > 1");
        if (!workspace || workspace_bytes < (int64_t)split_k * n_img * H * W * Cout * 4 || !fmc_aligned16(workspace))
            FMC_FAIL(FMC_E_SHAPE, "conv3x3_halo4: split_k %d needs a 16-byte aligned workspace of %lld bytes", split_k, (long long)split_k * n_img * H * W * Cout * 4);
    }
    C4Params P;
    P.x = (const bf16_t*)x; P.x2 = (const bf16_t*)x2; P.c1 = Cin1;
    P.w = (const bf16_t*)w_packed; P.bias = (const bf16_t*)bias; P.temb = (const bf16_t*)temb; P.res = (const bf16_t*)residual; P.out = (bf16_t*)out;
    P.n_img = n_img; P.H = H; P.W = W; P.cin = Cin; P.cout = Cout; P.ups = upsample2x ? 1 : 0;
    P.temb_ld = temb_row_stride; P.temb_div = temb ? temb_img_div : 1;
    P.gn_part = gn_partials; P.tiles_n = Cout / BN;
    P.splits = split_k; P.ws = (float*)workspace;
    const int64_t hs = upsample2x ? H / 2 : H, ws = upsample2x ? W / 2 : W;
    P.x_bytes = (int64_t)n_img * hs * ws * Cin1 * 2; P.x2_bytes = (int64_t)n_img * hs * ws * (Cin - Cin1) * 2;
    P.w_bytes = (int64_t)Cout * 9 * Cin * 2;
    hipStream_t st = (hipStream_t)stream;
    if (c4_tw(W) == 8) launch_c4<8, 4>(P, st);
    else if (wide) launch_c4<16, 8>(P, st);
    else launch_c4<16, 4>(P, st);
    FMC_CHECK_LAUNCH("fmc_conv3x3_halo4_bf16");
    return 0;
}
```

### synfmc_amd/hip_ops.py

```python
from __future__ import annotations

import atexit
import math
import os
from typing import Optional, Tuple

import torch

from . import _lib
from ._lib import FMC_BF16, FMC_F32

_DT = {torch.bfloat16: FMC_BF16, torch.float32: FMC_F32}


def _dt(t: torch.Tensor) -> int:
    try:
        return _DT[t.dtype]
    except KeyError:
        raise TypeError(f"fmc kernels take bf16 or fp32 activations, got {t.dtype}") from None


def _dev(*ts: torch.Tensor) -> None:
    for t in ts:
        if t is not None and not t.is_cuda:
# ... 1484 lines not shown
            and groups == 32 and gn_tag[1] == C and gn_tag[0].shape[0] == n_img and gn_tag[0].shape[1] <= 64 and gn_tag[0].shape[2] == groups
            and hw % 160 == 0 and C % 64 == 0 and N % 320 == 0 and (M // 160) * (N // 320) >= _cus(x.device) and n_img * N * C * 2 <= GN_FOLD_MAX_BYTES
            and M * max(C, N) * 2 < (1 << 31) and (ln is None or (LN_EPILOGUE and ln.stats_only and N == 320))
            and os.environ.get("FMC_G160_PERSIST", "1") != "0")


def linear_gnfold(x: torch.Tensor, gn_tag, gamma: torch.Tensor, beta: torch.Tensor, groups: int, eps: float, weight: torch.Tensor, bias,
                  ln: Optional[LnSpec] = None) -> torch.Tensor:
    part = gn_tag[0]
    _dev(x, part, gamma, beta, weight, bias)
    n_img, hw, C = x.shape
    N = weight.shape[0]
    M = n_img * hw
    lib = _lib.load()
    w_img = torch.empty(n_img, N, C, dtype=torch.bfloat16, device=x.device)
    b_img = torch.empty(n_img, N, dtype=torch.float32, device=x.device)
    gn_epilogue_calls["consumed"] += 1
    _lib.check(lib.fmc_groupnorm_fold_linear(part.data_ptr(), int(part.shape[1]), gamma.data_ptr(), beta.data_ptr(), weight.data_ptr(), _p(bias),
                                             w_img.data_ptr(), b_img.data_ptr(), n_img, hw, C, int(groups), N, float(eps), int(W_TILEMAJOR), _stream()),
               "fmc_groupnorm_fold_linear")
    out = torch.empty(n_img, hw, N, dtype=x.dtype, device=x.device)
    stats = None
    if ln is not None:
        stats = torch.empty(M, 2, dtype=torch.float32, device=x.device)
        ln_epilogue_calls["emitted"] += 1
    _log_call("own_linear", (M, N, C, "gn-fold", 0), 2.0 * M * N * C)
    _lib.check(lib.fmc_linear_bf16_imgw(x.data_ptr(), w_img.data_ptr(), b_img.data_ptr(), out.data_ptr(), M, N, C, C, N, hw, _p(stats),
                                        float(ln.eps) if ln is not None else 0.0, int(W_TILEMAJOR), _stream()), "fmc_linear_bf16_imgw")
    if ln is not None:
        out._fmc_ln = (stats, ln.key, True)
    return out


FF_BLOCKED = os.environ.get("FMC_FF_BLOCKED", "1") != "0"


def ff_blocked_ok(x: torch.Tensor, w1_il160: Optional[torch.Tensor], w2: torch.Tensor, residual) -> bool:
    if not FF_BLOCKED or w1_il160 is None or torch.is_grad_enabled():
        return False
    N1, Kd = w1_il160.shape
    N2, Cff = w2.shape
    M = x.numel() // x.shape[-1]
    return (x.is_cuda and x.dtype == torch.bfloat16 and w1_il160.dtype == torch.bfloat16 and w2.dtype == torch.bfloat16 and x.is_contiguous()
            and w1_il160.is_contiguous() and w2.is_contiguous() and N1 == 2 * Cff and Cff % 160 == 0 and N2 % 320 == 0 and Kd % 64 == 0
            and M % 160 == 0 and M >= 16384 and (M // 160) * (N1 // 320) > _cus(x.device) and M * Cff * 2 < (1 << 31)
            and (residual is None or (residual.is_contiguous() and residual.dtype == x.dtype))
            and os.environ.get("FMC_G160_PERSIST", "1") != "0")


def geglu_linear_blocked(x: torch.Tensor, weight_il160: torch.Tensor, bias_il160) -> torch.Tensor:
    pend = getattr(x, "_fmc_pending_ln", None)
    N, Kd = weight_il160.shape
    M = x.numel() // Kd
    out = torch.empty(*x.shape[:-1], N // 2, dtype=x.dtype, device=x.device)
    if pend is not None:
        stats, gamma, beta, _ = pend
        wg, c, b = _ln_folded_weight(weight_il160, bias_il160, gamma, beta)
        _dev(x, wg, c, b, stats)
        ln_epilogue_calls["consumed"] += 1
        wt = _w_tilemajor(wg) if W_TILEMAJOR else wg
        args = (wt.data_ptr(), None, None, out.data_ptr(), M, N, Kd, 0, 1.0, 1, 0, 1, stats.data_ptr(), c.data_ptr(), b.data_ptr(), int(W_TILEMAJOR))
    else:
        _dev(x, weight_il160, bias_il160)
        wt = _w_tilemajor(weight_il160) if W_TILEMAJOR else weight_il160
        args = (wt.data_ptr(), _p(bias_il160), None, out.data_ptr(), M, N, Kd, 0, 1.0, 1, 0, 1, None, None, None, int(W_TILEMAJOR))
    _log_call("own_linear", (M, N, Kd, "geglu-blocked", 0), 2.0 * M * N * Kd)
    _lib.check(_lib.load().fmc_linear_bf16_ffblk(x.data_ptr(), *args, _stream()), "fmc_linear_bf16_ffblk")
    return out


def linear_from_blocked(xb: torch.Tensor, weight: torch.Tensor, bias, residual, alpha: float = 1.0, out: Optional[torch.Tensor] = None) -> torch.Tensor:
    _dev(xb, weight, bias, residual, out)
    N, Kd = weight.shape
    M = xb.numel() // Kd
    if out is None:
        out = torch.empty(*xb.shape[:-1], N, dtype=xb.dtype, device=xb.device)
    assert out.is_contiguous() and out.numel() == M * N and out.dtype == xb.dtype
    wt = _w_tilemajor(weight) if W_TILEMAJOR else weight
    _log_call("own_linear", (M, N, Kd, "from-blocked", int(residual is not None)), 2.0 * M * N * Kd)
    _lib.check(_lib.load().fmc_linear_bf16_ffblk(xb.data_ptr(), wt.data_ptr(), _p(bias), _p(residual), out.data_ptr(), M, N, Kd,
                                                 0 if residual is None else N, float(alpha), 0, 1, 0, None, None, None, int(W_TILEMAJOR), _stream()),
               "fmc_linear_bf16_ffblk")
    return out


FF_TAIL = os.environ.get("FMC_FF_TAIL", "1") != "0"


def ff_tail_ok(h: torch.Tensor, w2: torch.Tensor, wp: torch.Tensor, tail_residual: Optional[torch.Tensor]) -> bool:
    C = h.shape[-1]
    M = h.numel() // C
    return (FF_TAIL and not torch.is_grad_enabled() and h.dtype == torch.bfloat16 and h.is_contiguous() and wp.dtype == torch.bfloat16 and w2.dtype == torch.bfloat16
            and wp.ndim == 2 and wp.shape[1] == w2.shape[0] == C and wp.shape[0] % 320 == 0 and C % 64 == 0 and w2.shape[1] % 64 == 0
            and M % 160 == 0 and (M // 160) * (wp.shape[0] // 320) >= _cus(h.device) and M * max(w2.shape[1], C) * 2 < (1 << 31)
            and tail_residual is not None and tail_residual.dtype == h.dtype and tail_residual.is_contiguous()
            and tail_residual.numel() == M * wp.shape[0] and os.environ.get("FMC_G160_PERSIST", "1") != "0")


def fold_ff_tail(w2: torch.Tensor, b2: Optional[torch.Tensor], wp: torch.Tensor, bp: Optional[torch.Tensor]):
    with torch.no_grad():
        wpf = wp.detach().float()
        wc = torch.cat([wpf @ w2.detach().float(), wpf], dim=1).to(torch.bfloat16).contiguous()
        bc = None
        if b2 is not None or bp is not None:
            bc = (wpf @ b2.detach().float()) if b2 is not None else torch.zeros(wp.shape[0], dtype=torch.float32, device=wp.device)
            if bp is not None:
                bc = bc + bp.detach().float()
            bc = bc.to(torch.bfloat16).contiguous()
    return wc, bc


def ff_tail(mid_blocked: torch.Tensor, h: torch.Tensor, w_cat: torch.Tensor, b_cat: Optional[torch.Tensor], tail_residual: torch.Tensor,
            gn_hw: int = 0) -> torch.Tensor:
    _dev(mid_blocked, h, w_cat, b_cat, tail_residual)
    N, Kd = w_cat.shape
    C = h.shape[-1]
    M = h.numel() // C
    assert mid_blocked.numel() == M * (Kd - C) and tail_residual.numel() == M * N
    out = torch.empty_like(tail_residual)
    part = None
    if gn_hw and gn_emit_ok(M, N, Kd, gn_hw, h.dtype):
        part = torch.empty(M // gn_hw, gn_hw // 160, 32, 2, dtype=torch.float32, device=h.device)
        gn_epilogue_calls["emitted"] += 1
    wt = _w_tilemajor(w_cat) if W_TILEMAJOR else w_cat
    _log_call("own_linear", (M, N, Kd, "ff-tail", 1), 2.0 * M * N * Kd)
    _lib.check(_lib.load().fmc_linear_bf16_fftail(mid_blocked.data_ptr(), h.data_ptr(), wt.data_ptr(), _p(b_cat), tail_residual.data_ptr(), out.data_ptr(),
                                                  M, N, Kd, Kd - C, C, N, _p(part), int(gn_hw if part is not None else 0), int(W_TILEMAJOR), _stream()),
               "fmc_linear_bf16_fftail")
    if part is not None:
        out._fmc_gn = (part, N)
    return out


def linear_gn(x: torch.Tensor, weight: torch.Tensor, bias, residual, alpha: float, residual2, hw: int):
    _dev(x, weight, bias, residual)
    N, Kd = weight.shape
    M, ldx = _rows2d(x)
    out = torch.empty(*x.shape[:-1], N, dtype=x.dtype, device=x.device)
    part = torch.empty(M // hw, hw // 160, 32, 2, dtype=torch.float32, device=x.device)
    ldres = 0 if residual is None else _rows2d(residual)[1]
    gn_epilogue_calls["emitted"] += 1
    wt = _w_tilemajor(weight) if W_TILEMAJOR else weight
    _log_call("own_linear", (M, N, Kd, "gn", (residual is not None) + (residual2 is not None)), 2.0 * M * N * Kd)
    _lib.check(_lib.load().fmc_linear_bf16_gn(x.data_ptr(), wt.data_ptr(), _p(bias), _p(residual), out.data_ptr(), M, N, Kd, ldx, ldres, N,
                                              float(alpha), _p(residual2), part.data_ptr(), int(hw), int(W_TILEMAJOR), _stream()), "fmc_linear_bf16_gn")
    out._fmc_gn = (part, N)
    return out


def conv3x3_gn(x_nhwc: torch.Tensor, weight_cl: torch.Tensor, bias, temb, residual_nhwc, temb_div: int, upsample: bool, stride2: bool):
    n, h, w, cin = x_nhwc.shape
    if upsample:
        h, w = 2 * h, 2 * w
    if stride2:
        h, w = h // 2, w // 2
    cout = weight_cl.shape[0]
    out = torch.empty(n, h, w, cout, dtype=x_nhwc.dtype, device=x_nhwc.device)
    part = torch.empty(n, (h * w) // 160, 32, 2, dtype=torch.float32, device=x_nhwc.device)
    gn_epilogue_calls["emitted"] += 1
    wt = _w_tilemajor_conv(weight_cl) if W_TILEMAJOR else weight_cl
    _lib.check(_lib.load().fmc_conv3x3_bf16_gn(x_nhwc.data_ptr(), wt.data_ptr(), _p(bias), _p(temb), _p(residual_nhwc), out.data_ptr(),
                                               n, h, w, cin, cout, 0 if temb is None else temb.stride(0), int(temb_div),
                                               2 if stride2 else int(upsample), part.data_ptr(), int(W_TILEMAJOR), _stream()), "fmc_conv3x3_bf16_gn")
    return out, (part, cout)


CONV_HALO = os.environ.get("FMC_CONV_HALO", "1") != "0"
CONV_HALO_MIN_TILES = int(os.environ.get("FMC_CONV_HALO_MIN_TILES", "200"))
LINEAR4 = os.environ.get("FMC_LINEAR4", "1") != "0"
CONV_HALO4 = os.environ.get("FMC_CONV_HALO4", "1") != "0"
CONV_GN_FUSED = os.environ.get("FMC_CONV_GN_FUSED", "0") == "1"
conv_halo_calls = {"conv": 0, "gn_fused": 0, "stats_pass": 0, "stats_from_producer": 0}


def conv3x3_halo_supported(n: int, h: int, w: int, cin: int, cin1: int, cout: int, upsample: bool) -> bool:
    return bool(_lib.load().fmc_conv3x3_halo_supported(n, h, w, cin, cin1, cout, int(upsample)))


def _w_halo_packed(weight_cl: torch.Tensor) -> torch.Tensor:
    cache = _owner_cache(weight_cl, "_fmc_wtm")
    key = ("halo", weight_cl.storage_offset(), tuple(weight_cl.shape), tuple(weight_cl.stride()), weight_cl._version)
    hit = cache.get(key)
    if hit is None:
        cout, cin = weight_cl.shape[:2]
        assert weight_cl.is_contiguous(memory_format=torch.channels_last)
        hit = torch.empty(cout * 9 * cin, dtype=weight_cl.dtype, device=weight_cl.device)
        _lib.check(_lib.load().fmc_conv3x3_halo_pack_weight(weight_cl.data_ptr(), hit.data_ptr(), cin, cout, _stream()), "fmc_conv3x3_halo_pack_weight")
        cache[key] = hit
    return hit


def groupnorm_coef(partials: torch.Tensor, gamma: torch.Tensor, beta: torch.Tensor, hw: int, C: int, groups: int, eps: float,
                   want_stats: bool = False):
    _dev(partials, gamma, beta)
    N, splits, G, _ = partials.shape
    assert G == groups and partials.dtype == torch.float32 and partials.is_contiguous() and gamma.dtype == torch.float32
    coef = torch.empty(N, C, 2, dtype=torch.float32, device=partials.device)
    stats = torch.empty(N, G, 2, dtype=torch.float32, device=partials.device) if want_stats else None
    _lib.check(_lib.load().fmc_groupnorm_coef(partials.data_ptr(), splits, gamma.data_ptr(), beta.data_ptr(), coef.data_ptr(), _p(stats), N, hw, C,
                                              groups, float(eps), _stream()), "fmc_groupnorm_coef")
    return (coef, stats) if want_stats else coef


def conv3x3_halo4_supported(n: int, h: int, w: int, cin: int, cin1: int, cout: int, upsample: bool, wide: bool = False) -> bool:
    return bool(_lib.load().fmc_conv3x3_halo4_supported(n, h, w, cin, cin1, cout, int(upsample), int(wide)))


def _w_halo4_packed(weight_cl: torch.Tensor, wide: bool = False) -> torch.Tensor:
    cache = _owner_cache(weight_cl, "_fmc_wtm")
    key = ("halo4w" if wide else "halo4", weight_cl.storage_offset(), tuple(weight_cl.shape), tuple(weight_cl.stride()), weight_cl._version)
    hit = cache.get(key)
    if hit is None:
        cout, cin = weight_cl.shape[:2]
        assert weight_cl.is_contiguous(memory_format=torch.channels_last)
        hit = torch.empty(cout * 9 * cin, dtype=weight_cl.dtype, device=weight_cl.device)
        _lib.check(_lib.load().fmc_conv3x3_halo4_pack_weight(weight_cl.data_ptr(), hit.data_ptr(), cin, cout, int(wide), _stream()),
                   "fmc_conv3x3_halo4_pack_weight")
        cache[key] = hit
    return hit


def conv3x3_halo4_split(n: int, h: int, w: int, cin: int, cout: int, cus: int = 256, wide: bool = False) -> int:
    tiles = _lib.load().fmc_conv3x3_halo4_tiles(n, h, w, cout, int(wide))
    if tiles >= (3 * cus) // 4:
        return 1
    nchunk = cin // 64
    best = 1
    for s in range(2, min(nchunk, 16) + 1):
        if nchunk % s == 0 and tiles * s <= cus + cus // 8:
            best = s
    return best


def conv3x3_halo4(x_nhwc: torch.Tensor, weight_cl: torch.Tensor, bias=None, temb=None, residual_nhwc=None, temb_div: int = 1, upsample: bool = False,
                  x2_nhwc: Optional[torch.Tensor] = None, emit_gn: bool = False, split_k: Optional[int] = None, wide: bool = False):
    _dev(x_nhwc, weight_cl, bias, temb, residual_nhwc, x2_nhwc)
    n, hs, ws, c1 = x_nhwc.shape
    h, w = (2 * hs, 2 * ws) if upsample else (hs, ws)
    cout, cin = weight_cl.shape[:2]
    assert x_nhwc.is_contiguous() and x_nhwc.dtype == torch.bfloat16 and weight_cl.dtype == torch.bfloat16
    if x2_nhwc is not None:
        assert x2_nhwc.is_contiguous() and x2_nhwc.shape[:3] == x_nhwc.shape[:3] and x2_nhwc.dtype == x_nhwc.dtype and c1 + x2_nhwc.shape[3] == cin
    else:
        assert c1 == cin
    assert temb is None or (temb.stride(1) == 1 and temb.shape == (n // temb_div, cout) and n % temb_div == 0)
    assert residual_nhwc is None or (residual_nhwc.is_contiguous() and residual_nhwc.shape == (n, h, w, cout))
    L = _lib.load()
    wp = _w_halo4_packed(weight_cl, wide)
    out = torch.empty(n, h, w, cout, dtype=x_nhwc.dtype, device=x_nhwc.device)
    if split_k is None:
        split_k = 1 if emit_gn else conv3x3_halo4_split(n, h, w, cin, cout, wide=wide)
    ws, ws_bytes = (None, 0) if split_k <= 1 else _splitk_workspace(x_nhwc.device, split_k, n * h * w, cout)
    part = torch.empty(n, L.fmc_conv3x3_halo4_row_blocks_per_image(h, w), 32, 2, dtype=torch.float32, device=x_nhwc.device) if emit_gn else None
    conv_halo_calls["conv4"] = conv_halo_calls.get("conv4", 0) + 1
    if call_log is not None:
        call_log.append(("conv_halo4", (n, h, w, cin, cout, bool(upsample)), 2.0 * n * h * w * cout * 9 * cin))
    _lib.check(L.fmc_conv3x3_halo4_bf16(x_nhwc.data_ptr(), _p(x2_nhwc), c1, wp.data_ptr(), _p(bias), _p(temb), _p(residual_nhwc), out.data_ptr(),
                                        n, h, w, cin, cout, 0 if temb is None else temb.stride(0), int(temb_div), int(upsample), _p(part), int(split_k),
                                        ws, ws_bytes, int(wide), _stream()), "fmc_conv3x3_halo4_bf16")
    return (out, part) if emit_gn else out


def groupnorm_partials(x: torch.Tensor, groups: int, x2: Optional[torch.Tensor] = None) -> torch.Tensor:
    _dev(x, x2)
    N, S, C1 = x.shape
    C = C1 + (x2.shape[2] if x2 is not None else 0)
    assert x.is_contiguous() and (x2 is None or (x2.is_contiguous() and x2.shape[:2] == x.shape[:2] and x2.dtype == x.dtype))
    L = _lib.load()
    part = torch.empty(N, L.fmc_groupnorm_partial_splits(S, C), groups, 2, dtype=torch.float32, device=x.device)
    conv_halo_calls["stats_pass"] += 1
    _lib.check(L.fmc_groupnorm_partials(x.data_ptr(), _p(x2), C1 if x2 is not None else 0, part.data_ptr(), N, S, C, groups, _dt(x), _stream()),
               "fmc_groupnorm_partials")
    return part


def conv3x3_halo(x_nhwc: torch.Tensor, weight_cl: torch.Tensor, bias=None, temb=None, residual_nhwc=None, temb_div: int = 1, upsample: bool = False,
                 x2_nhwc: Optional[torch.Tensor] = None, gn_coef: Optional[torch.Tensor] = None, gn_act: bool = True, emit_gn: bool = False):
    _dev(x_nhwc, weight_cl, bias, temb, residual_nhwc, x2_nhwc, gn_coef)
    n, hs, ws, c1 = x_nhwc.shape
    h, w = (2 * hs, 2 * ws) if upsample else (hs, ws)
    cout, cin = weight_cl.shape[:2]
    assert x_nhwc.is_contiguous() and x_nhwc.dtype == torch.bfloat16 and weight_cl.dtype == torch.bfloat16
    if x2_nhwc is not None:
        assert x2_nhwc.is_contiguous() and x2_nhwc.shape[:3] == x_nhwc.shape[:3] and x2_nhwc.dtype == x_nhwc.dtype and c1 + x2_nhwc.shape[3] == cin
    else:
        assert c1 == cin
    assert temb is None or (temb.stride(1) == 1 and temb.shape == (n // temb_div, cout) and n % temb_div == 0)
    assert residual_nhwc is None or (residual_nhwc.is_contiguous() and residual_nhwc.shape == (n, h, w, cout))
    assert gn_coef is None or (gn_coef.shape == (n, cin, 2) and gn_coef.dtype == torch.float32 and gn_coef.is_contiguous())
    L = _lib.load()
    wp = _w_halo_packed(weight_cl)
    out = torch.empty(n, h, w, cout, dtype=x_nhwc.dtype, device=x_nhwc.device)
    part = torch.empty(n, L.fmc_conv3x3_halo_tiles_per_image(h, w), 32, 2, dtype=torch.float32, device=x_nhwc.device) if emit_gn else None
    conv_halo_calls["conv"] += 1
    conv_halo_calls["gn_fused"] += gn_coef is not None
    if call_log is not None:
        call_log.append(("conv_halo", (n, h, w, cin, cout, bool(upsample)), 2.0 * n * h * w * cout * 9 * cin))
    _lib.check(L.fmc_conv3x3_halo_bf16(x_nhwc.data_ptr(), _p(x2_nhwc), c1, wp.data_ptr(), _p(bias), _p(temb), _p(residual_nhwc), out.data_ptr(),
                                       n, h, w, cin, cout, 0 if temb is None else temb.stride(0), int(temb_div), int(upsample), _p(gn_coef),
                                       int(gn_act), _p(part), _stream()), "fmc_conv3x3_halo_bf16")
    return (out, part) if emit_gn else out


F32_GEMM = os.environ.get("FMC_F32_GEMM", "1") != "0"
f32_gemm_calls = {"linear": 0, "geglu": 0, "conv3x3": 0}


def split_bf16x3(src: torch.Tensor, role: int, dst: Optional[torch.Tensor] = None, col0: int = 0, K: Optional[int] = None) -> torch.Tensor:
    _dev(src)
    assert src.dtype == torch.float32
    C = src.shape[-1]
    rows, ld = _rows2d(src)
    K = C if K is None else K
    if dst is None:
        dst = torch.empty(rows, 3 * K, dtype=torch.bfloat16, device=src.device)
    assert dst.shape == (rows, 3 * K) and dst.is_contiguous()
    _lib.check(_lib.load().fmc_split_bf16x3(src.data_ptr(), dst.data_ptr(), rows, C, ld, 3 * K, col0, K, role, _stream()),
               "fmc_split_bf16x3")
    return dst


def _split_weight_cached(weight: torch.Tensor, rows: int, C: int) -> torch.Tensor:
    hit = getattr(weight, "_fmc_w3", None)
    if hit is None or hit[0] != (weight._version, weight.data_ptr()):
        w2 = weight.detach()
        w2 = w2.contiguous(memory_format=torch.channels_last).permute(0, 2, 3, 1).reshape(rows, C) if weight.ndim == 4 else w2.reshape(rows, C)
        hit = ((weight._version, weight.data_ptr()), split_bf16x3(w2.contiguous(), 1))
        try:
            weight._fmc_w3 = hit
        except Exception:
            pass
    return hit[1]


def _f32_arm(key_bf16, tile: int) -> int:
    if tile:
        return tile
    return _f32_arm_of(_choice.get(key_bf16, 0))


def _f32_arm_of(use: int) -> int:
    if ARM_160 <= use < ARM_160 + 5 or ARM_160B <= use < ARM_160B + 5 or use == ARM_256:
        return ARM_160
    if use >= 384:
        use -= 384
    elif use >= 256:
        use -= 256
    elif use >= 128:
        use -= 128
    if 16 <= use < 128:
        use &= 15
    return use if 1 <= use <= 14 else 0


def linear_f32(x: torch.Tensor, weight: torch.Tensor, bias=None, residual=None, alpha: float = 1.0, geglu: bool = False,
               tile: int = 0, split_k: int = 1, x2=None, residual2=None) -> torch.Tensor:
    tile, split_k = _decode_arm(tile, split_k)
    if split_k < 1:
        split_k = 1
    _dev(x, weight, bias, residual, x2)
    N, Kd = weight.shape
    M, _ = _rows2d(x)
    if x2 is None:
        x3 = split_bf16x3(x, 0)
    else:
        k1 = x.shape[-1]
        assert k1 + x2.shape[-1] == Kd and _rows2d(x2)[0] == M
        x3 = torch.empty(M, 3 * Kd, dtype=torch.bfloat16, device=x.device)
        split_bf16x3(x, 0, x3, 0, Kd)
        split_bf16x3(x2, 0, x3, k1, Kd)
    w3 = _split_weight_cached(weight, N, Kd)
    n_out = N // 2 if geglu else N
    out = torch.empty(*x.shape[:-1], n_out, dtype=torch.float32, device=x.device)
    ldres = 0
    if residual is not None:
        assert residual.shape == out.shape and residual.dtype == torch.float32
        _, ldres = _rows2d(residual)
    if residual2 is not None:
        assert residual is not None and residual2.shape == out.shape and _rows2d(residual2)[1] == ldres
    b = None if bias is None else bias.float()
    ws, ws_bytes = _splitk_workspace(x.device, split_k, M, N)
    f32_gemm_calls["geglu" if geglu else "linear"] += 1
    _lib.check(_lib.load().fmc_linear_x3_f32(x3.data_ptr(), w3.data_ptr(), _p(b), _p(residual), out.data_ptr(), M, N, 3 * Kd,
                                             3 * Kd, ldres, n_out, float(alpha), int(geglu), int(tile), int(split_k), ws, ws_bytes,
                                             _p(residual2), _stream()), "fmc_linear_x3_f32")
    return out


def conv3x3_f32(x_nhwc: torch.Tensor, weight: torch.Tensor, bias=None, temb=None, residual_nhwc=None, tile: int = 0,
                split_k: int = 1, temb_div: int = 1, upsample: bool = False, stride2: bool = False) -> torch.Tensor:
    tile, split_k = _decode_arm(tile, split_k)
    if split_k < 1:
        split_k = 1
    _dev(x_nhwc, weight, bias, temb, residual_nhwc)
    n, h, w, cin = x_nhwc.shape
    if upsample:
        h, w = 2 * h, 2 * w
    if stride2:
        assert not upsample and h % 2 == 0 and w % 2 == 0
        h, w = h // 2, w // 2
    cout = weight.shape[0]
    assert x_nhwc.is_contiguous() and x_nhwc.dtype == torch.float32
    assert temb is None or (temb.stride(1) == 1 and temb.shape == (n // temb_div, cout) and temb.dtype == torch.float32)
    assert residual_nhwc is None or (residual_nhwc.is_contiguous() and residual_nhwc.shape == (n, h, w, cout))
    x3 = split_bf16x3(x_nhwc.view(-1, cin), 0)
    w3 = _split_weight_cached(weight, cout * 9, cin)
    out = torch.empty(n, h, w, cout, dtype=torch.float32, device=x_nhwc.device)
    b = None if bias is None else bias.float()
    ws, ws_bytes = _splitk_workspace(x_nhwc.device, split_k, n * h * w, cout)
    f32_gemm_calls["conv3x3"] += 1
    _lib.check(_lib.load().fmc_conv3x3_x3_f32(x3.data_ptr(), w3.data_ptr(), _p(b), _p(temb), _p(residual_nhwc), out.data_ptr(),
                                              n, h, w, 3 * cin, cout, 0 if temb is None else temb.stride(0), int(temb_div),
                                              2 if stride2 else int(upsample), int(tile), int(split_k), ws, ws_bytes, _stream()),
               "fmc_conv3x3_x3_f32")
    return out


_choice = {}
_tune_log = {}
_calls = {}
AUTOTUNE = os.environ.get("FMC_AUTOTUNE", "1") != "0"
DETERMINISTIC = os.environ.get("FMC_DETERMINISTIC", "0") == "1"
_CACHE_ENV = os.environ.get("FMC_AUTOTUNE_CACHE", "")
_cache_state = {"loaded": False, "dirty": False, "meta": None}


def _cache_path():
    if _CACHE_ENV == "0":
        return None
    return _CACHE_ENV or os.path.join(os.path.dirname(_lib.LIB_PATH), "autotune_cache.json")


def _cache_meta():
    if _cache_state["meta"] is None:
        import hashlib
        with open(_lib.LIB_PATH, "rb") as f:
            sha = hashlib.sha256(f.read()).hexdigest()[:16]
        _cache_state["meta"] = {"lib_sha16": sha, "device": torch.cuda.get_device_name() if torch.cuda.is_available() else "cpu",
                                "arms": list(GEMM_TILES), "hipblaslt": vendor_version() if torch.cuda.is_available() else 0}
    return _cache_state["meta"]


DEFAULT_ARM_TABLE = os.path.join(os.path.dirname(os.path.abspath(__file__)), "autotune_default_mi355x.json")
stale_table_entries = [0]
autotune_sources = {"cache": 0, "defaults": 0}


def _load_table_file(path: str, strict_meta: bool) -> int:
    import ast
    import json
    if not path or not os.path.isfile(path):
        return 0
    try:
        with open(path) as f:
            blob = json.load(f)
        meta, mine = blob.get("meta") or {}, _cache_meta()
        if strict_meta and meta != mine:
            return 0
        if not strict_meta:
            arch = torch.cuda.get_device_properties(torch.cuda.current_device()).gcnArchName.split(":")[0]
            if meta.get("arch") != arch:
                return 0
        n = 0
        for k, v in blob["choices"].items():
            key = ast.literal_eval(k)
            if key[0] == "valgo" and meta.get("hipblaslt") != mine["hipblaslt"]:
                continue
            if key not in _choice:
                _choice[key] = int(v["arm"])
                _tune_log[key] = {int(a): ms for a, ms in v.get("ms", {}).items()}
                n += 1
        return n
    except Exception:
        return 0


def load_autotune_table(path: Optional[str] = None) -> int:
    _cache_state["loaded"] = True
    n = _load_table_file(path or _cache_path(), True)
    autotune_sources["cache"] += n
    if os.environ.get("FMC_AUTOTUNE_DEFAULTS", "1") != "0" and torch.cuda.is_available():
        d = _load_table_file(DEFAULT_ARM_TABLE, False)
        autotune_sources["defaults"] += d
        n += d
    return n


def save_autotune_table(path: Optional[str] = None) -> Optional[str]:
    import json
    path = path or _cache_path()
    if not path or not _choice:
        return None
    blob = {"meta": _cache_meta(),
            "choices": {repr(k): {"arm": v, "ms": _tune_log.get(k, {})} for k, v in _choice.items()}}
    tmp = f"{path}.{os.getpid()}.tmp"
    try:
        with open(tmp, "w") as f:
            json.dump(blob, f)
        os.replace(tmp, path)
    except OSError:
        return None
    _cache_state["dirty"] = False
    return path


def _save_at_exit():
    if _cache_state["dirty"] and os.environ.get("RANK", "0") == "0":
        save_autotune_table()


atexit.register(_save_at_exit)
GEMM_TILES = (1, 2, 3, 4, 5, 6, 7, 11,
              13,
              15,
              ARM_160B if W_TILEMAJOR else ARM_160,
              128 + 2, 128 + 3,
              128 + 13,
              256 + 13,
              384 + 13)
if os.environ.get("FMC_GEMM_ARMS"):
    GEMM_TILES = tuple(int(a) for a in os.environ["FMC_GEMM_ARMS"].split(","))


def autotune_report():
    return [(k, _choice[k], _tune_log.get(k, {}), _calls.get(k, 0)) for k in _choice]


_tune_stream = None
def _graph_ms(body, reps):
    g = torch.cuda.CUDAGraph()
    with torch.cuda.graph(g, stream=_tune_stream):
        for _ in range(reps):
            body()
    g.replay()
    _tune_stream.synchronize()
    ms = float("inf")
    for _ in range(3):
        e0, e1 = torch.cuda.Event(enable_timing=True), torch.cuda.Event(enable_timing=True)
        e0.record()
        g.replay()
        e1.record()
        _tune_stream.synchronize()
        ms = min(ms, e0.elapsed_time(e1) / reps)
    del g
    return ms


def _time_ms(fn, reps=8):
    global _tune_stream
    if _tune_stream is None:
        _tune_stream = torch.cuda.Stream()
    cur = torch.cuda.current_stream()
    _tune_stream.wait_stream(cur)
    with torch.cuda.stream(_tune_stream):
        fn()
        _tune_stream.synchronize()
        ms = _graph_ms(fn, reps)
    cur.wait_stream(_tune_stream)
    return ms


NO_VENDOR = os.environ.get("FMC_NO_VENDOR", "0") == "1"
dispatch_calls = {k: {"own": 0, "vendor": 0, "ineligible": 0} for k in ("linear", "geglu", "conv3x3")}
call_log = None


def _log_call(family: str, shape: tuple, flops: float) -> None:
    if call_log is not None:
        call_log.append((family, tuple(shape), float(flops)))


def _pick(key, hip_fn, lib_fn, static_hip: bool, extra_arms=(), k320: bool = False, own_only: bool = False) -> int:
    if not _cache_state["loaded"]:
        load_autotune_table()
    no_lib = (DETERMINISTIC and key[0] == "conv") or own_only or NO_VENDOR
    if no_lib:
        key = key + ("det",)
    use = _choice.get(key)
    _calls[key] = _calls.get(key, 0) + 1
    n320 = (key[5] if key[0] == "conv" else key[2]) % 320 == 0
    cands = tuple(t for t in GEMM_TILES + tuple(extra_arms)
                  if (t != 15 or k320)
                  and (not (ARM_160 <= t < ARM_160 + 5 or ARM_160B <= t < ARM_160B + 5 or t == ARM_256) or n320))
    if use is not None and not (use in cands or (use == 0 and not no_lib) or (use == -1 and key not in _tune_log)):
        _choice.pop(key, None)
        _tune_log.pop(key, None)
        stale_table_entries[0] += 1
        use = None
    if use is None:
        if not AUTOTUNE or torch.cuda.is_current_stream_capturing():
            return 0 if not (static_hip or no_lib) else -1
        times = ([] if no_lib else [(_time_ms(lib_fn), 0)]) + [(_time_ms(lambda t=t: hip_fn(t)), t) for t in cands]
        use = min(times)[1]
        _choice[key] = use
        _tune_log[key] = {arm: round(ms, 4) for ms, arm in times}
        _cache_state["dirty"] = True
    return use


def linear(x: torch.Tensor, weight: torch.Tensor, bias: Optional[torch.Tensor] = None,
           residual: Optional[torch.Tensor] = None, alpha: float = 1.0, x2: Optional[torch.Tensor] = None,
           residual2: Optional[torch.Tensor] = None, gn_hw: int = 0, ln: Optional["LnSpec"] = None,
           lazy_residual: bool = False) -> torch.Tensor:
    import torch.nn.functional as F
    pend = getattr(x, "_fmc_pending_ln", None)
    if pend is not None:
        if (x2 is None and residual is None and residual2 is None and alpha == 1.0 and not gn_hw and ln is None and weight.is_contiguous()
                and lnc_ok(x, weight)):
            dispatch_calls["linear"]["own"] += 1
            return linear_lnc(x, weight, bias, pend)
        x = resolve_pending_ln(x)

    def lib():
        xin = x if x2 is None else torch.cat([x, x2], dim=-1)
        if alpha == 1.0 and vendor_linear_ok(xin, weight, bias, residual):
            y = vendor_linear(xin, weight, bias, residual)
            return y if residual2 is None else y + residual2
        y = F.linear(xin, weight, bias)
        _log_call("vendor", (xin.numel() // xin.shape[-1], weight.shape[0], weight.shape[1], bias is not None, False), 2.0 * xin.numel() * weight.shape[0])
        if residual is not None:
            y = torch.add(residual, y, alpha=alpha)
            return y if residual2 is None else y + residual2
        return y if alpha == 1.0 else y * alpha

    N, Kd = weight.shape
    if (F32_GEMM and x.is_cuda and x.dtype == torch.float32 and weight.dtype == torch.float32 and Kd % 64 == 0 and N % 8 == 0
            and x.shape[-1] % 8 == 0 and (x.is_contiguous() or x.ndim == 2) and (x2 is None or x2.is_contiguous())
            and (residual is None or residual.dtype == torch.float32)):
        M = x.numel() // x.shape[-1]
        key = ("lin", M, N, Kd, bias is not None, (residual is not None) + (residual2 is not None), 0 if x2 is None else x.shape[-1])
        return linear_f32(x, weight, bias, residual, alpha, tile=_f32_arm(key, 0), x2=x2, residual2=residual2)
    ok = x.is_cuda and x.dtype == torch.bfloat16 and weight.dtype == torch.bfloat16 and Kd % 64 == 0 and N % 8 == 0
    if x2 is None:
        ok = ok and linear_supported(x, weight)
    else:
        ok = ok and x.shape[-1] % 64 == 0 and x2.dtype == x.dtype and x2.is_contiguous()
    if not ok or (x.ndim > 2 and not x.is_contiguous()):
        dispatch_calls["linear"]["ineligible"] += 1
        return lib()
    M = x.numel() // x.shape[-1]
    if ln is not None and x2 is None and not gn_hw and ln_emit_ok(x, weight, residual, residual2, ln):
        dispatch_calls["linear"]["own"] += 1
        return linear_ln(x, weight, bias, residual, alpha, residual2, ln)
    if (gn_hw and x2 is None and x.is_contiguous() and gn_emit_ok(M, N, Kd, gn_hw, x.dtype)
            and (residual is None or (residual.is_contiguous() and residual.dtype == x.dtype))
            and (residual2 is None or residual2.is_contiguous())):
        dispatch_calls["linear"]["own"] += 1
        return linear_gn(x, weight, bias, residual, alpha, residual2, gn_hw)
    key = ("lin", M, N, Kd, bias is not None, (residual is not None) + (residual2 is not None),
           0 if x2 is None else x.shape[-1])
    hip = lambda tile: (linear4_bf16(x, weight, bias, residual, alpha, residual2) if tile == ARM_G4
                        else linear_bf16(x, weight, bias, residual, alpha, tile=tile, x2=x2, residual2=residual2))
    small = (ARM_SMALLM, ARM_SMALLM + 2) if (M <= 2560 and x2 is None and residual2 is None) else ()
    t160 = ((M + 159) // 160) * ((N + 159) // 160)
    if (LINEAR4 and x2 is None and weight.is_contiguous() and 48 <= t160 <= 640 and Kd >= 320
            and _lib.load().fmc_linear4_supported(M, N, Kd, _rows2d(x)[1])
            and (residual is None or _rows2d(residual)[1] % 8 == 0)
            and (residual2 is None or (residual is not None and _rows2d(residual2)[1] == _rows2d(residual)[1]))):
        small = small + (ARM_G4,)
    use = _pick(key, hip, lib, Kd <= 640 and N <= 1024 and M >= 16384, split_arms(M, N, Kd) + small,
                k320=(Kd == 320 and N % 320 == 0 and M % 64 == 0 and x2 is None and residual2 is None))
    if (use == 0 and lazy_residual and LAZY_RESIDUAL and residual is not None and residual2 is None and alpha == 1.0 and x2 is None
            and N in (320, 640, 1280) and residual.is_contiguous() and not torch.is_grad_enabled()
            and not vendor_linear_ok(x, weight, bias, residual)):
        dispatch_calls["linear"]["vendor"] += 1
        y = F.linear(x, weight, bias)
        y._fmc_pending_add = residual
        return y
    dispatch_calls["linear"]["vendor" if use == 0 else "own"] += 1
    return lib() if use == 0 else hip(max(use, 0))


def geglu_linear(x: torch.Tensor, weight: torch.Tensor, bias, weight_il: torch.Tensor, bias_il, weight_il160=None,
                 bias_il160=None) -> torch.Tensor:
    import torch.nn.functional as F
    pend = getattr(x, "_fmc_pending_ln", None)
    if pend is not None:
        if weight_il160 is not None and weight_il160.is_contiguous() and lnc_ok(x, weight_il160):
            return linear_lnc(x, weight_il160, bias_il160, pend, geglu=True)
        x = resolve_pending_ln(x)
    lib = lambda: geglu(F.linear(x, weight, bias))
    if (F32_GEMM and x.is_cuda and x.dtype == torch.float32 and weight_il.dtype == torch.float32 and weight_il.shape[0] % 64 == 0
            and weight_il.shape[1] % 64 == 0 and x.is_contiguous()):
        N, Kd = weight.shape
        arm = _f32_arm(("geglu", x.numel() // Kd, N, Kd), 0)
        if arm in (ARM_160, ARM_160B) and weight_il160 is not None:
            return linear_f32(x, weight_il160, bias_il160, geglu=True, tile=ARM_160)
        return linear_f32(x, weight_il, bias_il, geglu=True, tile=0 if arm in (ARM_160, ARM_160B) else arm)
    if not linear_supported(x, weight_il) or weight_il.shape[0] % 64 or (x.ndim > 2 and not x.is_contiguous()):
        dispatch_calls["geglu"]["ineligible"] += 1
        return lib()
    N, Kd = weight.shape
    M = x.numel() // Kd
    has160 = weight_il160 is not None and N % 320 == 0

    def hip(tile):
        if tile in (ARM_160, ARM_256, ARM_160B):
            return linear_bf16(x, weight_il160, bias_il160, geglu=True, tile=tile) if has160 else linear_bf16(x, weight_il, bias_il, geglu=True, tile=13)
        return linear_bf16(x, weight_il, bias_il, geglu=True, tile=tile)
    use = _pick(("geglu", M, N, Kd), hip, lib, M >= 65536)
    dispatch_calls["geglu"]["vendor" if use == 0 else "own"] += 1
    return lib() if use == 0 else hip(max(use, 0))


def conv3x3(x_nchw: torch.Tensor, weight_cl: torch.Tensor, bias, temb=None, residual_nchw=None, stride=(1, 1),
            padding=(1, 1), temb_div: int = 1, upsample: bool = False, emit_gn: bool = False, own_only: bool = False) -> torch.Tensor:
    import torch.nn.functional as F

    def lib():
        xin = F.interpolate(x_nchw, scale_factor=2.0, mode="nearest") if upsample else x_nchw
        y = F.conv2d(xin, weight_cl, bias, stride, padding)
        if temb is not None:
            y = y + (temb if temb_div == 1 else temb.repeat_interleave(temb_div, dim=0))[:, :, None, None]
        if residual_nchw is not None:
            y = y + residual_nchw
        return y

    if (F32_GEMM and x_nchw.is_cuda and x_nchw.dtype == torch.float32 and weight_cl.dtype == torch.float32
            and tuple(weight_cl.shape[2:]) == (3, 3) and tuple(padding) == (1, 1) and weight_cl.shape[1] % 64 == 0
            and weight_cl.shape[0] % 8 == 0 and (tuple(stride) == (1, 1) or (tuple(stride) == (2, 2) and not upsample
                                                                           and x_nchw.shape[-1] % 2 == 0 and x_nchw.shape[-2] % 2 == 0))):
        n, cin, h, w = x_nchw.shape
        x = x_nchw.permute(0, 2, 3, 1)
        r = None if residual_nchw is None else residual_nchw.permute(0, 2, 3, 1)
        if x.is_contiguous() and (r is None or r.is_contiguous()) and (temb is None or temb.stride(1) == 1):
            s2 = tuple(stride) == (2, 2)
            ho, wo = (2 * h, 2 * w) if upsample else ((h // 2, w // 2) if s2 else (h, w))
            key = ("conv", n, ho, wo, cin, weight_cl.shape[0], temb is not None, r is not None, upsample, s2)
            return conv3x3_f32(x, weight_cl, bias, temb, r, tile=_f32_arm(key, 0), temb_div=temb_div, upsample=upsample,
                               stride2=s2).permute(0, 3, 1, 2)
    if not conv3x3_supported(x_nchw, weight_cl, stride, padding):
        dispatch_calls["conv3x3"]["ineligible"] += 1
        return lib()
    n, cin, h, w = x_nchw.shape
    cout = weight_cl.shape[0]
    x = x_nchw.permute(0, 2, 3, 1)
    r = None if residual_nchw is None else residual_nchw.permute(0, 2, 3, 1)
    if not x.is_contiguous() or (r is not None and not r.is_contiguous()):
        dispatch_calls["conv3x3"]["ineligible"] += 1
        return lib()
    if upsample:
        h, w = 2 * h, 2 * w
    stride2 = tuple(stride) == (2, 2)
    if stride2:
        h, w = h // 2, w // 2
    if (CONV_HALO and not stride2 and (temb is None or temb.stride(1) == 1) and conv3x3_halo_supported(n, h, w, cin, cin, cout, upsample)
            and n * _lib.load().fmc_conv3x3_halo_tiles_per_image(h, w) * (cout // 160) >= CONV_HALO_MIN_TILES):
        want = bool(emit_gn and GN_EPILOGUE and cout % 64 == 0 and 160 % (cout // 32) == 0 and not torch.is_grad_enabled())
        dispatch_calls["conv3x3"]["own"] += 1
        y = conv3x3_halo(x, weight_cl, bias, temb, r, temb_div, upsample, emit_gn=want)
        if want:
            y, part = y
            gn_epilogue_calls["emitted"] += 1
            y = y.permute(0, 3, 1, 2)
            y._fmc_gn = (part, cout)
            return y
        return y.permute(0, 3, 1, 2)
    if (CONV_HALO and CONV_HALO4 and not stride2 and w % 8 == 0 and (temb is None or temb.stride(1) == 1)
            and conv3x3_halo4_supported(n, h, w, cin, cin, cout, upsample)
            and _lib.load().fmc_conv3x3_halo4_tiles(n, h, w, cout, 0) * conv3x3_halo4_split(n, h, w, cin, cout) >= CONV_HALO_MIN_TILES):
        dispatch_calls["conv3x3"]["own"] += 1
        want = bool(emit_gn and GN_EPILOGUE and h * w >= GN_MIN_HW and cout % 64 == 0 and 80 % (cout // 32) == 0 and not torch.is_grad_enabled()
                    and conv3x3_halo4_split(n, h, w, cin, cout) == 1)
        y = conv3x3_halo4(x, weight_cl, bias, temb, r, temb_div, upsample, emit_gn=want)
        if want:
            y, part = y
            gn_epilogue_calls["emitted"] += 1
            y = y.permute(0, 3, 1, 2)
            y._fmc_gn = (part, cout)
            return y
        return y.permute(0, 3, 1, 2)
    if emit_gn and gn_emit_ok(n * h * w, cout, 9 * cin, h * w, x.dtype):
        dispatch_calls["conv3x3"]["own"] += 1
        y, tag = conv3x3_gn(x, weight_cl, bias, temb, r, temb_div, upsample, stride2)
        y = y.permute(0, 3, 1, 2)
        y._fmc_gn = tag
        return y
    key = ("conv", n, h, w, cin, cout, temb is not None, r is not None, upsample, stride2)
    hip = lambda tile: conv3x3_bf16(x, weight_cl, bias, temb, r, tile=tile, temb_div=temb_div,
                                    upsample=upsample, stride2=stride2).permute(0, 3, 1, 2)
    tiles = ((n * h * w + 127) // 128) * ((cout + 127) // 128)
    use = _pick(key, hip, lib, tiles >= 256, split_arms(n * h * w, cout, 9 * cin), own_only=own_only)
    dispatch_calls["conv3x3"]["vendor" if use == 0 else "own"] += 1
    return lib() if use == 0 else hip(max(use, 0))


def _flipped_filter(weight_cl: torch.Tensor) -> torch.Tensor:
    hit = getattr(weight_cl, "_fmc_flipped", None)
    if hit is None or hit[0] != weight_cl._version:
        hit = (weight_cl._version,
               weight_cl.detach().flip(2, 3).permute(1, 0, 2, 3).contiguous(memory_format=torch.channels_last))
        weight_cl._fmc_flipped = hit
    return hit[1]


class _Conv3x3Frozen(torch.autograd.Function):
    @staticmethod
    def forward(ctx, x, weight_cl, bias, temb, residual, temb_div):
        ctx.save_for_backward(weight_cl)
        ctx.has_res = residual is not None and residual.requires_grad
        with torch.no_grad():
            return conv3x3(x, weight_cl, bias, temb, residual, (1, 1), (1, 1), temb_div)

    @staticmethod
    def backward(ctx, dy):
        (weight_cl,) = ctx.saved_tensors
        dy = dy.contiguous(memory_format=torch.channels_last)
        dx = None
        if ctx.needs_input_grad[0]:
            with torch.no_grad():
                dx = conv3x3(dy, _flipped_filter(weight_cl), None)
        return dx, None, None, None, (dy if ctx.has_res else None), None


def conv3x3_frozen(x, weight_cl, bias, temb=None, residual=None, temb_div: int = 1):
    return _Conv3x3Frozen.apply(x, weight_cl, bias, temb, residual, temb_div)


def _transposed_weight(weight: torch.Tensor) -> torch.Tensor:
    owner = weight._base if weight._base is not None else weight
    key = (weight.storage_offset(), tuple(weight.shape), tuple(weight.stride()), weight._version, weight.dtype)
    cache = getattr(owner, "_fmc_wt", None)
    if cache is None or cache[0] != owner._version:
        cache = (owner._version, {})
        try:
            owner._fmc_wt = cache
        except Exception:
            pass
    hit = cache[1].get(key)
    if hit is None:
        hit = weight.detach().t().contiguous()
        cache[1][key] = hit
    return hit


def linear_backward_data(dy: torch.Tensor, weight: torch.Tensor, alpha: float = 1.0) -> torch.Tensor:
    if dy.is_cuda and dy.dtype == torch.bfloat16 and weight.dtype == torch.bfloat16 and weight.shape[0] % 64 == 0 \
            and weight.shape[1] % 8 == 0:
        with torch.no_grad():
            return linear(dy if dy.is_contiguous() else dy.contiguous(), _transposed_weight(weight), None, None, alpha)
    dx = torch.matmul(dy, weight)
    return dx if alpha == 1.0 else dx * alpha


class _LinearFrozen(torch.autograd.Function):
    @staticmethod
    def forward(ctx, x, weight, bias, residual, alpha):
        ctx.save_for_backward(weight)
        ctx.alpha = alpha
        ctx.has_res = residual is not None and residual.requires_grad
        with torch.no_grad():
            return linear(x, weight, bias, residual, alpha)

    @staticmethod
    def backward(ctx, dy):
        (weight,) = ctx.saved_tensors
        dx = linear_backward_data(dy, weight, ctx.alpha) if ctx.needs_input_grad[0] else None
        return dx, None, None, (dy if ctx.has_res else None), None


def linear_frozen(x, weight, bias=None, residual=None, alpha: float = 1.0):
    return _LinearFrozen.apply(x, weight, bias, residual, alpha)


def column_sum(x: torch.Tensor, alpha: float = 1.0, out: Optional[torch.Tensor] = None, accumulate: bool = False) -> torch.Tensor:
    _dev(x, out)
    M, ld = _rows2d(x)
    N = x.shape[-1]
    if out is None:
        out, accumulate = torch.empty(N, dtype=torch.float32, device=x.device), False
    assert out.dtype == torch.float32 and out.is_contiguous() and out.numel() == N
    lib = _lib.load()
    ws = _workspace(x.device, lib.fmc_column_sum_workspace_bytes(M, N))
    _lib.check(lib.fmc_column_sum(x.data_ptr(), out.data_ptr(), M, N, ld, float(alpha), int(accumulate), ws.data_ptr(), _dt(x), _stream()),
               "fmc_column_sum")
    return out


class _LinearTrainable(torch.autograd.Function):

    @staticmethod
    def forward(ctx, x, weight, bias, residual, w_run, b_run):
        with torch.no_grad():
            y = linear(x, w_run, b_run, residual)
        ctx.save_for_backward(x, w_run)
        ctx.has_res = residual is not None and residual.requires_grad
        ctx.dtypes = (weight.dtype, None if bias is None else bias.dtype)
        return y

    @staticmethod
    def backward(ctx, dy):
        x, w_run = ctx.saved_tensors
        dy = dy if dy.dtype == x.dtype else dy.to(x.dtype)
        dy = dy if dy.is_contiguous() else dy.contiguous()
        N, Kd = w_run.shape
        dy2 = dy.view(-1, N)
        x2 = x if (x.ndim == 2 and not x.is_contiguous()) else x.reshape(-1, Kd)
        dx = dw = db = None
        with torch.no_grad():
            if ctx.needs_input_grad[0]:
                dx = linear_backward_data(dy, w_run).view(x.shape)
            if ctx.needs_input_grad[1]:
                dw = linear_wgrad(dy2, x2).to(ctx.dtypes[0])
            if ctx.needs_input_grad[2]:
                db = column_sum(dy2).to(ctx.dtypes[1])
        return dx, dw, db, (dy if ctx.has_res else None), None, None


def linear_trainable(x: torch.Tensor, weight: torch.Tensor, bias: Optional[torch.Tensor] = None, residual: Optional[torch.Tensor] = None,
                     w_run: Optional[torch.Tensor] = None, b_run: Optional[torch.Tensor] = None) -> torch.Tensor:
    if w_run is None:
        w_run = weight.detach() if weight.dtype == x.dtype else weight.detach().to(x.dtype)
    if b_run is None and bias is not None:
        b_run = bias.detach() if bias.dtype == x.dtype else bias.detach().to(x.dtype)
    return _LinearTrainable.apply(x, weight, bias, residual, w_run, b_run)


def conv3x3_weight_grad(x_nhwc: torch.Tensor, dy_nhwc: torch.Tensor) -> torch.Tensor:
    _dev(x_nhwc, dy_nhwc)
    n, H, W, cin = x_nhwc.shape
    cout = dy_nhwc.shape[-1]
    assert dy_nhwc.shape[:3] == x_nhwc.shape[:3] and x_nhwc.is_contiguous() and dy_nhwc.is_contiguous()
    assert x_nhwc.dtype == torch.bfloat16 and dy_nhwc.dtype == torch.bfloat16 and cin % 8 == 0 and cout % 8 == 0
    Hp, Wp = H + 2, (W + 2 + 7) // 8 * 8
    Lk = (n * Hp * Wp + 63) // 64 * 64
    G = Wp + 8
    Lg = Lk + 2 * G
    lib = _lib.load()
    xt = torch.empty(3, cin, Lg, dtype=torch.bfloat16, device=x_nhwc.device)
    dyt = torch.empty(cout, Lk, dtype=torch.bfloat16, device=x_nhwc.device)
    _lib.check(lib.fmc_nhwc_to_cmajor_padded(x_nhwc.data_ptr(), xt.data_ptr(), n, H, W, cin, Lg, G, 3, _stream()),
               "fmc_nhwc_to_cmajor_padded")
    _lib.check(lib.fmc_nhwc_to_cmajor_padded(dy_nhwc.data_ptr(), dyt.data_ptr(), n, H, W, cout, Lk, 0, 1, _stream()),
               "fmc_nhwc_to_cmajor_padded")
    rows = xt.view(3 * cin, Lg)
    tiles = ((3 * cin + 127) // 128) * ((cout + 127) // 128)
    split = 1
    while split < 16 and tiles * split * 2 <= 512 and Lk // 64 >= split * 4:
        split *= 2
    out = []
    for dy in range(3):
        xs = rows[:, G + (dy - 1) * Wp: G + (dy - 1) * Wp + Lk]
        out.append(linear_bf16(xs, dyt, None, None, 1.0, tile=1, split_k=split))
    dwt = torch.stack(out)
    return dwt.view(3, 3, cin, cout).permute(3, 2, 0, 1)


class _Conv3x3Trainable(torch.autograd.Function):

    @staticmethod
    def forward(ctx, x, weight, bias):
        ctx.save_for_backward(x, weight)
        ctx.has_bias = bias is not None
        with torch.no_grad():
            w_cl = weight.detach().to(x.dtype).contiguous(memory_format=torch.channels_last)
            b = None if bias is None else bias.detach().to(x.dtype)
            return conv3x3(x, w_cl, b)

    @staticmethod
    def backward(ctx, dy):
        x, weight = ctx.saved_tensors
        dy = dy.contiguous(memory_format=torch.channels_last)
        dx = dw = db = None
        with torch.no_grad():
            if ctx.needs_input_grad[0]:
                w_flip = weight.detach().to(dy.dtype).flip(2, 3).permute(1, 0, 2, 3).contiguous(memory_format=torch.channels_last)
                dx = conv3x3(dy, w_flip, None)
            if ctx.needs_input_grad[1]:
                dw = conv3x3_weight_grad(x.permute(0, 2, 3, 1), dy.permute(0, 2, 3, 1)).to(weight.dtype)
            if ctx.has_bias and ctx.needs_input_grad[2]:
                db = dy.sum(dim=(0, 2, 3), dtype=torch.float32).to(weight.dtype)
        return dx, dw, (db if ctx.has_bias else None)


def conv3x3_trainable(x, weight, bias=None):
    return _Conv3x3Trainable.apply(x, weight, bias)


import ctypes as _ct


class WgradProblem(_ct.Structure):
    _fields_ = [("a", _ct.c_void_p), ("b", _ct.c_void_p), ("out", _ct.c_void_p), ("M", _ct.c_int64), ("lda", _ct.c_int64),
                ("ldb", _ct.c_int64), ("ldo", _ct.c_int64), ("N", _ct.c_int), ("K", _ct.c_int), ("alpha", _ct.c_float), ("accumulate", _ct.c_int)]


_wgrad_ws = {}


def linear_wgrad_group(problems):
    outs, descs = [], []
    for a, b, alpha, out, acc in problems:
        _dev(a, b, out)
        (M, lda), (Mb, ldb) = _rows2d(a), _rows2d(b)
        N, Kd = a.shape[-1], b.shape[-1]
        assert M == Mb, "linear_wgrad: a and b must have the same rows"
        if out is None:
            out = torch.empty(N, Kd, dtype=torch.float32, device=a.device)
            acc = False
        assert out.dtype == torch.float32 and out.ndim == 2 and out.shape == (N, Kd) and out.stride(1) == 1
        outs.append(out)
        if a.dtype != torch.bfloat16 or b.dtype != torch.bfloat16:
            g = torch.matmul(a.reshape(M, N).t().float(), b.reshape(M, Kd).float())
            out.add_(g, alpha=alpha) if acc else torch.mul(g, alpha, out=out)
            continue
        descs.append(WgradProblem(a.data_ptr(), b.data_ptr(), out.data_ptr(), M, lda, ldb, out.stride(0), N, Kd, float(alpha), int(bool(acc))))
    if not descs:
        return outs
    lib = _lib.load()
    arr = (WgradProblem * len(descs))(*descs)
    need = lib.fmc_linear_wgrad_workspace_bytes(arr, len(descs))
    if need < 0:
        _lib.check(-1, "fmc_linear_wgrad_bf16")
    ws, ws_bytes = None, 0
    if need > 0:
        dev = outs[0].device
        key = (dev.index, torch.cuda.current_stream().cuda_stream)
        buf = _wgrad_ws.get(key)
        if buf is None or buf.numel() * 4 < need:
            if buf is not None:
                _ws_retired.append(buf)
            buf = torch.empty(need // 4 + 1024, dtype=torch.float32, device=dev)
            _wgrad_ws[key] = buf
        ws, ws_bytes = buf.data_ptr(), buf.numel() * 4
    _log_call("lora_wgrad", tuple((d.M, d.N, d.K) for d in descs), sum(2.0 * d.M * d.N * d.K for d in descs))
    _lib.check(lib.fmc_linear_wgrad_bf16(arr, len(descs), ws, ws_bytes, _stream()), "fmc_linear_wgrad_bf16")
    return outs


def linear_wgrad(a: torch.Tensor, b: torch.Tensor, alpha: float = 1.0, out: Optional[torch.Tensor] = None,
                 accumulate: bool = False) -> torch.Tensor:
    return linear_wgrad_group([(a, b, alpha, out, accumulate)])[0]


def _lora_gemm(x, weight, bias=None, residual=None, x2=None, out=None):
    if x.dtype == torch.bfloat16 and x.is_cuda:
        return linear_bf16(x, weight, bias, residual, x2=x2, out=out)
    xin = x if x2 is None else torch.cat([x, x2], dim=-1)
    y = torch.nn.functional.linear(xin, weight, bias)
    if residual is not None:
        y = y + residual
    if out is None:
        return y
    out.copy_(y)
    return out


def lora_pad_rank(r: int, dtype) -> int:
# ... 103 lines not shown
```

Before: 38.49 steps/s.

## Fold nearest-upsample into 3x3 conv via four-phase 2x2 subpixel weights

Adds a phase mode to both halo conv kernels. A nearest-2x upsample followed by a 3x3 conv becomes four 2x2 convolutions on the low-resolution input, using pre-summed folded weights, with each phase writing interleaved output pixels. This cuts the MAC count per output from 9 taps to 4 and avoids reading the upsampled activation. The trade-offs are weight folding done in bf16 via fp32 accumulation, which adds rounding differences, a cached 16-tap packed weight copy, and a restricted dispatch (no temb or residual, inference only).

```diff
diff --git a/include/fmc_hip.h b/include/fmc_hip.h
--- a/include/fmc_hip.h
+++ b/include/fmc_hip.h
@@ -135,6 +135,14 @@
 int fmc_conv3x3_halo4_bf16(const void* x, const void* x2, int Cin1, const void* w_packed, const void* bias, const void* temb, const void* residual,
                            void* out, int n_img, int H, int W, int Cin, int Cout, int64_t temb_row_stride, int temb_img_div, int upsample2x,
                            float* gn_partials, int split_k, void* workspace, int64_t workspace_bytes, int wide, void* stream);
+int64_t fmc_conv3x3_upfold_packed_bytes(int Cin, int Cout);
+int fmc_conv3x3_upfold_pack_weight(const void* w, void* dst, int Cin, int Cout, int tile_channels, void* stream);
+int fmc_conv3x3_halo_fold_supported(int n_img, int Hs, int Ws, int Cin, int Cout);
+int fmc_conv3x3_halo_fold_bf16(const void* x, const void* w_folded, const void* bias, void* out, int n_img, int Hs, int Ws, int Cin, int Cout,
+                               float* gn_partials, void* stream);
+int fmc_conv3x3_halo4_fold_supported(int n_img, int Hs, int Ws, int Cin, int Cout, int wide);
+int fmc_conv3x3_halo4_fold_bf16(const void* x, const void* w_folded, const void* bias, void* out, int n_img, int Hs, int Ws, int Cin, int Cout,
+                                float* gn_partials, int wide, void* stream);
 int fmc_groupnorm_coef(const float* partials, int part_splits, const float* gamma, const float* beta, float* coef, float* stats, int N, int HW,
                        int C, int G, float eps, void* stream);
 
diff --git a/synfmc_amd/_lib.py b/synfmc_amd/_lib.py
--- a/synfmc_amd/_lib.py
+++ b/synfmc_amd/_lib.py
@@ -71,6 +71,12 @@
     "fmc_conv3x3_halo4_tiles": (c_int, [c_int, c_int, c_int, c_int, c_int]),
     "fmc_conv3x3_halo4_bf16": (c_int, [c_void_p, c_void_p, c_int, c_void_p, c_void_p, c_void_p, c_void_p, c_void_p, c_int, c_int, c_int, c_int, c_int,
                                        c_int64, c_int, c_int, c_void_p, c_int, c_void_p, c_int64, c_int, c_void_p]),
+    "fmc_conv3x3_upfold_packed_bytes": (c_int64, [c_int, c_int]),
+    "fmc_conv3x3_upfold_pack_weight": (c_int, [c_void_p, c_void_p, c_int, c_int, c_int, c_void_p]),
+    "fmc_conv3x3_halo_fold_supported": (c_int, [c_int, c_int, c_int, c_int, c_int]),
+    "fmc_conv3x3_halo_fold_bf16": (c_int, [c_void_p, c_void_p, c_void_p, c_void_p, c_int, c_int, c_int, c_int, c_int, c_void_p, c_void_p]),
+    "fmc_conv3x3_halo4_fold_supported": (c_int, [c_int, c_int, c_int, c_int, c_int, c_int]),
+    "fmc_conv3x3_halo4_fold_bf16": (c_int, [c_void_p, c_void_p, c_void_p, c_void_p, c_int, c_int, c_int, c_int, c_int, c_void_p, c_int, c_void_p]),
     "fmc_linear4_supported": (c_int, [c_int64, c_int, c_int, c_int64]),
     "fmc_vendor_linear_candidates": (c_int, [c_int64, c_int, c_int, c_int64, c_int64, c_int64, c_int, c_int]),
     "fmc_vendor_linear_bf16": (c_int, [c_void_p, c_void_p, c_void_p, c_void_p, c_void_p, c_int64, c_int, c_int, c_int64, c_int64, c_int64, c_int, c_void_p,
diff --git a/synfmc_amd/csrc/conv_halo.hip b/synfmc_amd/csrc/conv_halo.hip
--- a/synfmc_amd/csrc/conv_halo.hip
+++ b/synfmc_amd/csrc/conv_halo.hip
@@ -35,7 +35,9 @@
 
 constexpr int nh(int i) { return (i >= 0 && i <= 12 && (i & 1) == 0) ? 1 : 0; }
 
-template <int GN>
+constexpr int nhp(int i) { return (i >= 0 && i <= 3) ? (i < 3 ? 2 : 1) : 0; }
+
+template <int GN, bool PH = false>
 __global__ __launch_bounds__(512, 2)
 void conv_halo_kernel(const CHParams P) {
     extern __shared__ __attribute__((aligned(16))) unsigned char smem_raw[];
@@ -57,8 +59,11 @@
     const int tpi = P.tiles_y * P.tiles_x;
     const int img = tile_p / tpi, tin = tile_p - img * tpi;
     const int y0 = (tin / P.tiles_x) * TH, x0 = (tin % P.tiles_x) * TW;
-    const int n0 = tile_n * BN;
-    const int nchunk = P.cin >> 6, nsub = nchunk * 18;
+    constexpr int NS = PH ? 8 : 18;
+    const int tn1 = P.cout / BN;
+    const int phase = PH ? tile_n / tn1 : 0, py = phase >> 1, px_ = phase & 1;
+    const int n0 = (tile_n - phase * tn1) * BN;
+    const int nchunk = P.cin >> 6, nsub = nchunk * NS;
 
     const int Hs = P.ups ? P.H >> 1 : P.H, Ws = P.ups ? P.W >> 1 : P.W;
     const int pp = lane & 7, pg = ((lane & 7) + (lane >> 3)) & 7;
@@ -139,7 +144,7 @@
 #pragma unroll
     for (int mb = 0; mb < 5; ++mb) {
         const int idx = wr * 80 + mb * 16 + l15, ty = idx >> 5, tx = idx & 31;
-        afrag[mb] = kq * PLANE + (ty * HWID + tx) * 16;
+        afrag[mb] = kq * PLANE + (ty * HWID + tx) * 16 + (PH ? (py * HWID + px_) * 16 : 0);
     }
 
     {
@@ -174,8 +179,51 @@
         int cbuf = 0;
         float coef_next = 0.f;
         u32x4 hpk = {0u, 0u, 0u, 0u};
+        u32x4 hregp[3][2];
         for (int c = 0; c < nchunk; ++c) {
             const int abase = cbuf * HALO, nbuf = cbuf ^ 1;
+            if constexpr (PH) {
+                static_assert(!PH || GN == 0, "the phase mode has no GroupNorm operand path");
+                auto subp = [&](auto ic) {
+                    constexpr int i = decltype(ic)::value;
+                    constexpr int tap = i >> 1, hk = i & 1, ta = tap >> 1, tb = tap & 1;
+                    constexpr int aimm = hk * 4 * PLANE + (ta * HWID + tb) * 16;
+                    if constexpr (nhp(i - 3) >= 1) halo_store(2 * (i - 3), nbuf, hregp[(i - 3) % 3][0]);
+                    if constexpr (nhp(i - 3) == 2) halo_store(2 * (i - 3) + 1, nbuf, hregp[(i - 3) % 3][1]);
+                    {
+                        const unsigned char* Wp = smem_raw + wfrag + rd_slot * WSUB;
+#pragma unroll
+                        for (int nb = 0; nb < 5; ++nb) wf[nb] = __builtin_bit_cast(bf16x8, *reinterpret_cast<const u32x4*>(Wp + nb * 1024));
+#pragma unroll
+                        for (int mb = 0; mb < 5; ++mb)
+                            af[mb] = __builtin_bit_cast(bf16x8, *reinterpret_cast<const u32x4*>(smem_raw + abase + afrag[mb] + aimm));
+                        rd_slot = rd_slot + 1 == NBW ? 0 : rd_slot + 1;
+                    }
+                    if constexpr (nhp(i) >= 1) halo_load(2 * i, c + 1, hregp[i % 3][0]);
+                    if constexpr (nhp(i) == 2) halo_load(2 * i + 1, c + 1, hregp[i % 3][1]);
+                    w_issue(cls);
+                    {
+                        constexpr int extra = nhp(i - 1) + nhp(i);
+                        asm volatile("s_waitcnt vmcnt(%0)" ::"n"(2 * NW + extra) : "memory");
+                    }
+                    __builtin_amdgcn_sched_barrier(0);
+                    __builtin_amdgcn_s_barrier();
+                    __builtin_amdgcn_sched_barrier(0);
+                    __builtin_amdgcn_s_setprio(1);
+#pragma unroll
+                    for (int mb = 0; mb < 5; ++mb)
+#pragma unroll
+                        for (int nb = 0; nb < 5; ++nb)
+                            acc[mb][nb] = __builtin_amdgcn_mfma_f32_16x16x32_bf16(wf[nb], af[mb], acc[mb][nb], 0, 0, 0);
+                    __builtin_amdgcn_s_setprio(0);
+                    __builtin_amdgcn_sched_barrier(0);
+                    __builtin_amdgcn_s_barrier();
+                    __builtin_amdgcn_sched_barrier(0);
+                };
+                subp(IC<0>{}); subp(IC<1>{}); subp(IC<2>{}); subp(IC<3>{}); subp(IC<4>{}); subp(IC<5>{}); subp(IC<6>{}); subp(IC<7>{});
+                cbuf = nbuf;
+                continue;
+            }
             auto sub = [&](auto ic) {
                 constexpr int i = decltype(ic)::value;
                 constexpr int tap = i >> 1, hk = i & 1, ky = tap / 3, kx = tap % 3;
@@ -237,7 +285,10 @@
     bf16_t* Os = reinterpret_cast<bf16_t*>(smem_raw);
     constexpr int CPR = BN / 8;
     const int vrows = min(TH, P.H - y0) * TW;
-    auto row_pixel = [&](int r) -> int64_t { return ((int64_t)img * P.H + y0 + (r >> 5)) * P.W + x0 + (r & 31); };
+    auto row_pixel = [&](int r) -> int64_t {
+        if constexpr (PH) return ((int64_t)img * (2 * P.H) + 2 * (y0 + (r >> 5)) + py) * (2 * P.W) + 2 * (x0 + (r & 31)) + px_;
+        return ((int64_t)img * P.H + y0 + (r >> 5)) * P.W + x0 + (r & 31);
+    };
     {
         u32x2 bt[5], tt[5];
         if (P.bias) {
@@ -326,7 +377,7 @@
         if (tid < GT) {
             float a = 0.f, b = 0.f;
             for (int k = 0; k < RP; ++k) { a += red[2 * (tid + k * GT)]; b += red[2 * (tid + k * GT) + 1]; }
-            float* dst = P.gn_part + (((int64_t)img * tpi + tin) * 32 + (n0 / cpg + tid)) * 2;
+            float* dst = P.gn_part + ((PH ? ((int64_t)img * tpi + tin) * 4 + phase : (int64_t)img * tpi + tin) * 32 + (n0 / cpg + tid)) * 2;
             dst[0] = a;
             dst[1] = b;
         }
@@ -347,6 +398,33 @@
         const int lc = p ^ (3 * ((row >> 3) & 1));
         const int64_t src = (((int64_t)(nt * BN + row) * 9 + tap) * cin + ch64 * 64 + hk * 32 + lc * 8);
         *reinterpret_cast<u32x4*>(dst + id * 8) = *reinterpret_cast<const u32x4*>(w + src);
+    }
+}
+
+__global__ __launch_bounds__(256) void conv_upfold_pack_kernel(const bf16_t* __restrict__ w, bf16_t* __restrict__ dst, int cout, int cin, int BN) {
+    const int64_t total = (int64_t)cout * 16 * cin / 8;
+    const int nchunk = cin >> 6, tn1 = cout / BN;
+    for (int64_t id = (int64_t)blockIdx.x * blockDim.x + threadIdx.x; id < total; id += (int64_t)gridDim.x * blockDim.x) {
+        int64_t t = id;
+        const int p = (int)(t & 3); t >>= 2;
+        const int row = (int)(t % BN); t /= BN;
+        const int hk = (int)(t & 1); t >>= 1;
+        const int tap = (int)(t & 3); t >>= 2;
+        const int ch64 = (int)(t % nchunk); t /= nchunk;
+        const int nt = (int)(t % tn1), phase = (int)(t / tn1);
+        const int py = phase >> 1, px = phase & 1, ta = tap >> 1, tb = tap & 1;
+        const int ky0 = py == 0 ? ta : 2 * ta, ky1 = py == 0 ? 2 * ta : ta + 1;
+        const int kx0 = px == 0 ? tb : 2 * tb, kx1 = px == 0 ? 2 * tb : tb + 1;
+        const int lc = p ^ (3 * ((row >> 3) & 1));
+        float v[8] = {0.f, 0.f, 0.f, 0.f, 0.f, 0.f, 0.f, 0.f};
+        for (int ky = ky0; ky <= ky1; ++ky)
+            for (int kx = kx0; kx <= kx1; ++kx) {
+                float f[8];
+                Vec8<bf16_t>::unpack(Vec8<bf16_t>::load_raw(w + (((int64_t)(nt * BN + row) * 9 + ky * 3 + kx) * cin + ch64 * 64 + hk * 32 + lc * 8)), f);
+#pragma unroll
+                for (int k = 0; k < 8; ++k) v[k] += f[k];
+            }
+        Vec8<bf16_t>::store(dst + id * 8, v);
     }
 }
 
@@ -444,6 +522,57 @@
     return 0;
 }
 
+extern "C" int64_t fmc_conv3x3_upfold_packed_bytes(int Cin, int Cout) { return (int64_t)Cout * 16 * Cin * 2; }
+
+extern "C" int fmc_conv3x3_upfold_pack_weight(const void* w, void* dst, int Cin, int Cout, int tile_channels, void* stream) {
+    if (!w || !dst) FMC_FAIL(FMC_E_NULL, "conv3x3_upfold_pack_weight: NULL pointer");
+    if ((tile_channels != 80 && tile_channels != 160) || Cin % 64 || Cout % tile_channels)
+        FMC_FAIL(FMC_E_SHAPE, "conv3x3_upfold_pack_weight: tile_channels 80 / 160, Cin %% 64, Cout %% tile_channels (Cin=%d Cout=%d tile=%d)", Cin, Cout, tile_channels);
+    if (!fmc_aligned16(w) || !fmc_aligned16(dst)) FMC_FAIL(FMC_E_ALIGN, "conv3x3_upfold_pack_weight: pointers must be 16-byte aligned");
+    const int64_t chunks = (int64_t)Cout * 16 * Cin / 8;
+    const int grid = (int)((chunks + 255) / 256 < 4096 ? (chunks + 255) / 256 : 4096);
+    hipLaunchKernelGGL(conv_upfold_pack_kernel, dim3(grid), dim3(256), 0, (hipStream_t)stream, (const bf16_t*)w, (bf16_t*)dst, Cout, Cin, tile_channels);
+    FMC_CHECK_LAUNCH("fmc_conv3x3_upfold_pack_weight");
+    return 0;
+}
+
+extern "C" int fmc_conv3x3_halo_fold_supported(int n_img, int Hs, int Ws, int Cin, int Cout) {
+    if (!fmc_conv3x3_halo_supported(n_img, Hs, Ws, Cin, Cin, Cout, 0)) return 0;
+    if ((int64_t)Cout * 16 * Cin * 2 >= (1ll << 31)) return 0;
+    if ((int64_t)n_img * Hs * Ws * 4 >= (1ll << 31)) return 0;
+    return 1;
+}
+
+extern "C" int fmc_conv3x3_halo_fold_bf16(const void* x, const void* w_folded, const void* bias, void* out, int n_img, int Hs, int Ws, int Cin,
+                                          int Cout, float* gn_partials, void* stream) {
+    if (!x || !w_folded || !out) FMC_FAIL(FMC_E_NULL, "conv3x3_halo_fold: NULL x / w / out");
+    if (!fmc_conv3x3_halo_fold_supported(n_img, Hs, Ws, Cin, Cout))
+        FMC_FAIL(FMC_E_SHAPE, "conv3x3_halo_fold: needs Ws %% 32 == 0, Cin %% 64 == 0, Cout %% 160 == 0, operands < 2 GiB (n=%d Hs=%d Ws=%d Cin=%d Cout=%d)",
+                 n_img, Hs, Ws, Cin, Cout);
+    if (!fmc_aligned16(x) || !fmc_aligned16(w_folded) || !fmc_aligned16(out) || (bias && (reinterpret_cast<uintptr_t>(bias) & 7)))
+        FMC_FAIL(FMC_E_ALIGN, "conv3x3_halo_fold: x / w / out must be 16-byte aligned, bias 8-byte aligned");
+    if (gn_partials && (Cout % 64 || BN % (Cout / 32)))
+        FMC_FAIL(FMC_E_SHAPE, "conv3x3_halo_fold: the statistics epilogue needs Cout %% 64 == 0 and 160 %% (Cout / 32) == 0 (Cout=%d)", Cout);
+    CHParams P;
+    P.x = (const bf16_t*)x; P.x2 = nullptr; P.c1 = Cin;
+    P.w = (const bf16_t*)w_folded; P.bias = (const bf16_t*)bias; P.temb = nullptr; P.res = nullptr; P.out = (bf16_t*)out;
+    P.n_img = n_img; P.H = Hs; P.W = Ws; P.cin = Cin; P.cout = Cout; P.ups = 0;
+    P.temb_ld = 0; P.temb_div = 1;
+    P.gn_coef = nullptr; P.gn_act = 0; P.gn_part = gn_partials;
+    P.tiles_y = (Hs + TH - 1) / TH; P.tiles_x = Ws / TW; P.tiles_n = 4 * (Cout / BN);
+    P.x_bytes = (int64_t)n_img * Hs * Ws * Cin * 2; P.x2_bytes = 0;
+    P.w_bytes = (int64_t)Cout * 16 * Cin * 2;
+    static FmcPerDeviceFlag raised;
+    if (!raised) {
+        (void)hipFuncSetAttribute(reinterpret_cast<const void*>(&conv_halo_kernel<0, true>), hipFuncAttributeMaxDynamicSharedMemorySize, LDS_BYTES);
+        raised = true;
+    }
+    const unsigned grid = (unsigned)(n_img * P.tiles_y * P.tiles_x * P.tiles_n);
+    hipLaunchKernelGGL((conv_halo_kernel<0, true>), dim3(grid), dim3(512), LDS_BYTES, (hipStream_t)stream, P);
+    FMC_CHECK_LAUNCH("fmc_conv3x3_halo_fold_bf16");
+    return 0;
+}
+
 extern "C" int fmc_conv3x3_halo_tiles_per_image(int H, int W) { return ((H + TH - 1) / TH) * (W / TW); }
 
 extern "C" int fmc_groupnorm_coef(const float* partials, int part_splits, const float* gamma, const float* beta, float* coef, float* stats,
diff --git a/synfmc_amd/csrc/conv_halo4.hip b/synfmc_amd/csrc/conv_halo4.hip
--- a/synfmc_amd/csrc/conv_halo4.hip
+++ b/synfmc_amd/csrc/conv_halo4.hip
@@ -45,12 +45,13 @@
 
 template <int I> using IC = std::integral_constant<int, I>;
 
-template <int NPIECE> constexpr int pps() { return NPIECE > 12 ? 2 : 1; }
-template <int NPIECE> constexpr int nh(int i) {
-    return (i >= 0 && pps<NPIECE>() * i < NPIECE) ? (pps<NPIECE>() == 2 && 2 * i + 1 < NPIECE ? 2 : 1) : 0;
-}
-
-template <int TW, int NWV>
+template <int NPIECE, bool PH> constexpr int pps() { return PH ? (NPIECE + 3) / 4 : (NPIECE > 12 ? 2 : 1); }
+template <int NPIECE, bool PH> constexpr int nh(int i) {
+    constexpr int S = pps<NPIECE, PH>();
+    return (i >= 0 && S * i < NPIECE) ? (NPIECE - S * i < S ? NPIECE - S * i : S) : 0;
+}
+
+template <int TW, int NWV, bool PH = false>
 __global__ __launch_bounds__(64 * NWV, NWV / 4)
 void conv_halo4_kernel(const C4Params P) {
     using G = Geo<TW, NWV>;
@@ -84,11 +85,14 @@
             tile_n = lin - tile_p * P.tiles_n;
         }
     }
-    const int n0 = tile_n * BN;
+    constexpr int NS = PH ? 8 : 18;
+    const int tn1 = P.cout / BN;
+    const int phase = PH ? tile_n / tn1 : 0, py = phase >> 1, px_ = phase & 1;
+    const int n0 = (tile_n - phase * tn1) * BN;
     const int nchunk_all = P.cin >> 6;
     const int per = (nchunk_all + P.splits - 1) / P.splits;
     const int ck0 = split * per, nchunk = max(0, min(nchunk_all, ck0 + per) - ck0);
-    const int nsub = max(nchunk, 1) * 18;
+    const int nsub = max(nchunk, 1) * NS;
     const int tpi = P.tiles_y * P.tiles_x;
     const int rb0 = tile_p * NB, rb_total = P.n_img * tpi;
 
@@ -128,7 +132,7 @@
     };
 
     const unsigned w_vo0 = (unsigned)(lane * 16 + wave * 1024);
-    const int w_base = (tile_n * nchunk_all + ck0) * 18 * WSUB;
+    const int w_base = (tile_n * nchunk_all + ck0) * NS * WSUB;
     int iss_soff = w_base, iss_left = nsub, iss_slot = 0;
     auto w_issue = [&](auto cls) {
         unsigned char* dst = smem_raw + OFF_W + iss_slot * WSUB + wave * 1024;
@@ -147,7 +151,7 @@
 #pragma unroll
     for (int mb = 0; mb < 5; ++mb) {
         const int idx = wp * 80 + mb * 16 + l15, blk = idx / RB, r = idx - blk * RB, ty = r / TW, tx = r - ty * TW;
-        afrag[mb] = kq * PLANE + (blk * HB + ty * HW_ + tx) * 16;
+        afrag[mb] = kq * PLANE + (blk * HB + ty * HW_ + tx) * 16 + (PH ? (py * HW_ + px_) * 16 : 0);
     }
 
     {
@@ -161,7 +165,7 @@
 
     auto main_loop = [&](auto cls) {
         constexpr int NW = decltype(cls)::value ? 2 : 1;
-        constexpr int PPS = pps<NPIECE>();
+        constexpr int PPS = pps<NPIECE, PH>();
         u32x4 hreg[3][PPS];
         w_issue(cls); w_issue(cls); w_issue(cls);
         if constexpr (DW == 4) w_issue(cls);
@@ -188,20 +192,20 @@
             const int abase = cbuf * HALO, nbuf = cbuf ^ 1;
             auto sub = [&](auto ic) {
                 constexpr int i = decltype(ic)::value;
-                constexpr int n1 = (i + 1) % 18, tap1 = n1 >> 1, hk1 = n1 & 1;
-                constexpr int aimm1 = hk1 * 4 * PLANE + ((tap1 / 3) * HW_ + (tap1 % 3)) * 16;
+                constexpr int n1 = (i + 1) % NS, tap1 = n1 >> 1, hk1 = n1 & 1;
+                constexpr int aimm1 = hk1 * 4 * PLANE + (PH ? (tap1 >> 1) * HW_ + (tap1 & 1) : (tap1 / 3) * HW_ + (tap1 % 3)) * 16;
                 {
-                    constexpr int extra = nh<NPIECE>(i - 1) + (DW == 4 ? nh<NPIECE>(i - 2) : 0);
+                    constexpr int extra = nh<NPIECE, PH>(i - 1) + (DW == 4 ? nh<NPIECE, PH>(i - 2) : 0);
                     asm volatile("s_waitcnt vmcnt(%0)" ::"n"((DW - 2) * NW + extra) : "memory");
                 }
                 __builtin_amdgcn_sched_barrier(0);
                 __builtin_amdgcn_s_barrier();
                 __builtin_amdgcn_sched_barrier(0);
-                if constexpr (nh<NPIECE>(i - 3) >= 1) halo_store(PPS * (i - 3), nbuf, hreg[(i - 3) % 3][0]);
-                if constexpr (nh<NPIECE>(i - 3) == 2) halo_store(PPS * (i - 3) + 1, nbuf, hreg[(i - 3) % 3][PPS - 1]);
-                read_frags((i + 1) & 1, i == 17 ? nbuf * HALO : abase, aimm1);
-                if constexpr (nh<NPIECE>(i) >= 1) hreg[i % 3][0] = halo_load(PPS * i, c + 1);
-                if constexpr (nh<NPIECE>(i) == 2) hreg[i % 3][PPS - 1] = halo_load(PPS * i + 1, c + 1);
+#pragma unroll
+                for (int k = 0; k < nh<NPIECE, PH>(i - 3); ++k) halo_store(PPS * (i - 3) + k, nbuf, hreg[(i + 15) % 3][k]);
+                read_frags((i + 1) & 1, i == NS - 1 ? nbuf * HALO : abase, aimm1);
+#pragma unroll
+                for (int k = 0; k < nh<NPIECE, PH>(i); ++k) hreg[i % 3][k] = halo_load(PPS * i + k, c + 1);
                 w_issue(cls);
 #pragma unroll
                 for (int mb = 0; mb < 5; ++mb)
@@ -209,8 +213,9 @@
                     for (int nb = 0; nb < 5; ++nb)
                         acc[mb][nb] = __builtin_amdgcn_mfma_f32_16x16x32_bf16(wf[i & 1][nb], af[i & 1][mb], acc[mb][nb], 0, 0, 0);
                 if constexpr (INTERLEAVE) {
-#pragma unroll
-                    for (int k = 0; k < 2; ++k) {
+                    constexpr int NST = PH ? PPS : 2, NRQ = PH ? PPS + 2 : 4;
+#pragma unroll
+                    for (int k = 0; k < NST; ++k) {
                         __builtin_amdgcn_sched_group_barrier(0x008, 1, 0);
                         __builtin_amdgcn_sched_group_barrier(0x200, 1, 0);
                     }
@@ -220,17 +225,20 @@
                         __builtin_amdgcn_sched_group_barrier(0x100, 1, 0);
                     }
 #pragma unroll
-                    for (int k = 0; k < 4; ++k) {
+                    for (int k = 0; k < NRQ; ++k) {
                         __builtin_amdgcn_sched_group_barrier(0x008, 1, 0);
                         __builtin_amdgcn_sched_group_barrier(0x020, 1, 0);
                     }
-                    __builtin_amdgcn_sched_group_barrier(0x008, 9, 0);
+                    __builtin_amdgcn_sched_group_barrier(0x008, 25 - 10 - NST - NRQ, 0);
                 }
                 __builtin_amdgcn_sched_barrier(0);
             };
             sub(IC<0>{}); sub(IC<1>{}); sub(IC<2>{}); sub(IC<3>{}); sub(IC<4>{}); sub(IC<5>{});
-            sub(IC<6>{}); sub(IC<7>{}); sub(IC<8>{}); sub(IC<9>{}); sub(IC<10>{}); sub(IC<11>{});
-            sub(IC<12>{}); sub(IC<13>{}); sub(IC<14>{}); sub(IC<15>{}); sub(IC<16>{}); sub(IC<17>{});
+            sub(IC<6>{}); sub(IC<7>{});
+            if constexpr (!PH) {
+                sub(IC<8>{}); sub(IC<9>{}); sub(IC<10>{}); sub(IC<11>{});
+                sub(IC<12>{}); sub(IC<13>{}); sub(IC<14>{}); sub(IC<15>{}); sub(IC<16>{}); sub(IC<17>{});
+            }
             cbuf = nbuf;
         }
     };
@@ -238,7 +246,7 @@
     asm volatile("s_waitcnt vmcnt(0) lgkmcnt(0)" ::: "memory");
     __syncthreads();
 
-    if (P.splits > 1) {
+    if (!PH && P.splits > 1) {
         const int64_t mtot = (int64_t)P.n_img * P.H * P.W;
 #pragma unroll
         for (int mb = 0; mb < 5; ++mb) {
@@ -260,6 +268,7 @@
         const int blk = r / RB, q = r - blk * RB, ty = q / TW, tx = q - ty * TW;
         const int rb = rb0 + blk, img = rb / tpi, rin = rb - img * tpi, yb = rin / P.tiles_x, xb = rin - yb * P.tiles_x, y = yb * TH + ty;
         ok = rb < rb_total && y < P.H;
+        if constexpr (PH) return ((int64_t)img * (2 * P.H) + 2 * y + py) * (2 * P.W) + 2 * (xb * TW + tx) + px_;
         return ((int64_t)img * P.H + y) * P.W + xb * TW + tx;
     };
     {
@@ -362,7 +371,7 @@
             if (tid < GT) {
                 float a = 0.f, b = 0.f;
                 for (int k = 0; k < RP; ++k) { a += red[2 * (tid + k * GT)]; b += red[2 * (tid + k * GT) + 1]; }
-                float* dst = P.gn_part + (((int64_t)img * tpi + sp) * 32 + (n0 / cpg + tid)) * 2;
+                float* dst = P.gn_part + ((PH ? ((int64_t)img * tpi + sp) * 4 + phase : (int64_t)img * tpi + sp) * 32 + (n0 / cpg + tid)) * 2;
                 dst[0] = a;
                 dst[1] = b;
             }
@@ -425,7 +434,7 @@
     }
 }
 
-template <int TW, int NWV> int launch_c4(C4Params& P, hipStream_t st) {
+template <int TW, int NWV, bool PH = false> int launch_c4(C4Params& P, hipStream_t st) {
     using G = Geo<TW, NWV>;
     P.tiles_y = (P.H + G::TH - 1) / G::TH;
     P.tiles_x = P.W / TW;
@@ -445,10 +454,10 @@
     }
     static FmcPerDeviceFlag raised;
     if (!raised) {
-        (void)hipFuncSetAttribute(reinterpret_cast<const void*>(&conv_halo4_kernel<TW, NWV>), hipFuncAttributeMaxDynamicSharedMemorySize, G::LDS_BYTES);
+        (void)hipFuncSetAttribute(reinterpret_cast<const void*>(&conv_halo4_kernel<TW, NWV, PH>), hipFuncAttributeMaxDynamicSharedMemorySize, G::LDS_BYTES);
         raised = true;
     }
-    hipLaunchKernelGGL((conv_halo4_kernel<TW, NWV>), dim3((unsigned)(P.tiles_p * P.tiles_n * P.splits)), dim3(G::NT), G::LDS_BYTES, st, P);
+    hipLaunchKernelGGL((conv_halo4_kernel<TW, NWV, PH>), dim3((unsigned)(P.tiles_p * P.tiles_n * P.splits)), dim3(G::NT), G::LDS_BYTES, st, P);
     if (P.splits > 1) {
         const int64_t chunks = (int64_t)P.n_img * P.H * P.W * (P.cout / 8);
         const unsigned grid = (unsigned)((chunks + 255) / 256 < 2048 ? (chunks + 255) / 256 : 2048);
@@ -532,3 +541,38 @@
     FMC_CHECK_LAUNCH("fmc_conv3x3_halo4_bf16");
     return 0;
 }
+
+extern "C" int fmc_conv3x3_halo4_fold_supported(int n_img, int Hs, int Ws, int Cin, int Cout, int wide) {
+    if (!fmc_conv3x3_halo4_supported(n_img, Hs, Ws, Cin, Cin, Cout, 0, wide)) return 0;
+    if ((int64_t)Cout * 16 * Cin * 2 >= (1ll << 31)) return 0;
+    if ((int64_t)n_img * Hs * Ws * 4 >= (1ll << 31)) return 0;
+    return 1;
+}
+
+extern "C" int fmc_conv3x3_halo4_fold_bf16(const void* x, const void* w_folded, const void* bias, void* out, int n_img, int Hs, int Ws, int Cin,
+                                           int Cout, float* gn_partials, int wide, void* stream) {
+    const int BN = wide ? 160 : 80;
+    if (!x || !w_folded || !out) FMC_FAIL(FMC_E_NULL, "conv3x3_halo4_fold: NULL x / w / out");
+    if (!fmc_conv3x3_halo4_fold_supported(n_img, Hs, Ws, Cin, Cout, wide))
+        FMC_FAIL(FMC_E_SHAPE, "conv3x3_halo4_fold: needs Ws %% 8 == 0 (wide: %% 16), Cin %% 64 == 0, Cout %% %d == 0, operands < 2 GiB "
+                 "(n=%d Hs=%d Ws=%d Cin=%d Cout=%d)", BN, n_img, Hs, Ws, Cin, Cout);
+    if (!fmc_aligned16(x) || !fmc_aligned16(w_folded) || !fmc_aligned16(out) || (bias && (reinterpret_cast<uintptr_t>(bias) & 7)))
+        FMC_FAIL(FMC_E_ALIGN, "conv3x3_halo4_fold: x / w / out must be 16-byte aligned, bias 8-byte aligned");
+    if (gn_partials && (Cout % 64 || BN % (Cout / 32)))
+        FMC_FAIL(FMC_E_SHAPE, "conv3x3_halo4_fold: the statistics epilogue needs Cout %% 64 == 0 and %d %% (Cout / 32) == 0 (Cout=%d)", BN, Cout);
+    C4Params P;
+    P.x = (const bf16_t*)x; P.x2 = nullptr; P.c1 = Cin;
+    P.w = (const bf16_t*)w_folded; P.bias = (const bf16_t*)bias; P.temb = nullptr; P.res = nullptr; P.out = (bf16_t*)out;
+    P.n_img = n_img; P.H = Hs; P.W = Ws; P.cin = Cin; P.cout = Cout; P.ups = 0;
+    P.temb_ld = 0; P.temb_div = 1;
+    P.gn_part = gn_partials; P.tiles_n = 4 * (Cout / BN);
+    P.splits = 1; P.ws = nullptr;
+    P.x_bytes = (int64_t)n_img * Hs * Ws * Cin * 2; P.x2_bytes = 0;
+    P.w_bytes = (int64_t)Cout * 16 * Cin * 2;
+    hipStream_t st = (hipStream_t)stream;
+    if (c4_tw(Ws) == 8) launch_c4<8, 4, true>(P, st);
+    else if (wide) launch_c4<16, 8, true>(P, st);
+    else launch_c4<16, 4, true>(P, st);
+    FMC_CHECK_LAUNCH("fmc_conv3x3_halo4_fold_bf16");
+    return 0;
+}
diff --git a/synfmc_amd/hip_ops.py b/synfmc_amd/hip_ops.py
--- a/synfmc_amd/hip_ops.py
+++ b/synfmc_amd/hip_ops.py
@@ -1810,6 +1810,102 @@
     return (out, part) if emit_gn else out
 
 
+UPS_FOLD = os.environ.get("FMC_UPS_FOLD", "1") != "0"
+UPS_FOLD_MIN_WS = int(os.environ.get("FMC_UPS_FOLD_MIN_WS", "8"))
+UPS_FOLD_WIDE = os.environ.get("FMC_UPS_FOLD_WIDE", "0") == "1"
+
+
+def upsample_fold_weights(weight: torch.Tensor) -> torch.Tensor:
+    rows = (((0,), (1, 2)), ((0, 1), (2,)))
+    cout, cin = weight.shape[:2]
+    wf = weight.new_zeros(2, 2, 2, 2, cout, cin)
+    for py in range(2):
+        for px in range(2):
+            for a in range(2):
+                for b in range(2):
+                    for ky in rows[py][a]:
+                        for kx in rows[px][b]:
+                            wf[py, px, a, b] += weight[:, :, ky, kx]
+    return wf
+
+
+def conv3x3_upfold_reference(x_nchw: torch.Tensor, wf: torch.Tensor, bias: Optional[torch.Tensor] = None) -> torch.Tensor:
+    import torch.nn.functional as F
+    n, _, hs, ws = x_nchw.shape
+    cout = wf.shape[4]
+    xp = F.pad(x_nchw, (1, 1, 1, 1))
+    out = x_nchw.new_zeros(n, cout, 2 * hs, 2 * ws)
+    for py in range(2):
+        for px in range(2):
+            k = wf[py, px].permute(2, 3, 0, 1)
+            out[:, :, py::2, px::2] = F.conv2d(xp[:, :, py:py + hs + 1, px:px + ws + 1], k)
+    return out if bias is None else out + bias[None, :, None, None]
+
+
+def conv3x3_upfold_arm(n: int, hs: int, ws: int, cin: int, cout: int) -> Optional[str]:
+    if not (UPS_FOLD and CONV_HALO) or ws < UPS_FOLD_MIN_WS:
+        return None
+    L = _lib.load()
+    if (L.fmc_conv3x3_halo_fold_supported(n, hs, ws, cin, cout)
+            and n * L.fmc_conv3x3_halo_tiles_per_image(hs, ws) * 4 * (cout // 160) >= CONV_HALO_MIN_TILES):
+        return "halo"
+    if not CONV_HALO4:
+        return None
+    wide = UPS_FOLD_WIDE and bool(L.fmc_conv3x3_halo4_fold_supported(n, hs, ws, cin, cout, 1))
+    if (L.fmc_conv3x3_halo4_fold_supported(n, hs, ws, cin, cout, int(wide))
+            and 4 * L.fmc_conv3x3_halo4_tiles(n, hs, ws, cout, int(wide)) >= CONV_HALO_MIN_TILES):
+        return "halo4w" if wide else "halo4"
+    return None
+
+
+def _w_upfold_packed(weight_cl: torch.Tensor, tile_channels: int) -> torch.Tensor:
+    cache = _owner_cache(weight_cl, "_fmc_wtm")
+    key = ("upfold%d" % tile_channels, weight_cl.storage_offset(), tuple(weight_cl.shape), tuple(weight_cl.stride()), weight_cl._version)
+    hit = cache.get(key)
+    if hit is None:
+        cout, cin = weight_cl.shape[:2]
+        assert weight_cl.is_contiguous(memory_format=torch.channels_last)
+        hit = torch.empty(cout * 16 * cin, dtype=weight_cl.dtype, device=weight_cl.device)
+        _lib.check(_lib.load().fmc_conv3x3_upfold_pack_weight(weight_cl.data_ptr(), hit.data_ptr(), cin, cout, tile_channels, _stream()),
+                   "fmc_conv3x3_upfold_pack_weight")
+        cache[key] = hit
+    return hit
+
+
+def conv3x3_upfold(x_nhwc: torch.Tensor, weight_cl: torch.Tensor, bias=None, emit_gn: bool = False, arm: Optional[str] = None):
+    _dev(x_nhwc, weight_cl, bias)
+    n, hs, ws, cin = x_nhwc.shape
+    cout = weight_cl.shape[0]
+    assert x_nhwc.is_contiguous() and x_nhwc.dtype == torch.bfloat16 and weight_cl.dtype == torch.bfloat16 and weight_cl.shape[1] == cin
+    assert not (torch.is_grad_enabled() and (x_nhwc.requires_grad or weight_cl.requires_grad)), "conv3x3_upfold: inference only"
+    if arm is None:
+        arm = conv3x3_upfold_arm(n, hs, ws, cin, cout)
+    if arm not in ("halo", "halo4", "halo4w"):
+        raise ValueError(f"conv3x3_upfold: no phase-mode launch for n={n} {hs}x{ws} {cin}->{cout} (arm {arm})")
+    L = _lib.load()
+    out = torch.empty(n, 2 * hs, 2 * ws, cout, dtype=x_nhwc.dtype, device=x_nhwc.device)
+    shape, flops = (n, 2 * hs, 2 * ws, cin, cout, True), 2.0 * n * 4 * hs * ws * cout * 9 * cin
+    conv_halo_calls["upfold"] = conv_halo_calls.get("upfold", 0) + 1
+    if arm == "halo":
+        wp = _w_upfold_packed(weight_cl, 160)
+        part = torch.empty(n, 4 * L.fmc_conv3x3_halo_tiles_per_image(hs, ws), 32, 2, dtype=torch.float32, device=x_nhwc.device) if emit_gn else None
+        conv_halo_calls["conv"] += 1
+        if call_log is not None:
+            call_log.append(("conv_halo", shape, flops))
+        _lib.check(L.fmc_conv3x3_halo_fold_bf16(x_nhwc.data_ptr(), wp.data_ptr(), _p(bias), out.data_ptr(), n, hs, ws, cin, cout, _p(part), _stream()),
+                   "fmc_conv3x3_halo_fold_bf16")
+    else:
+        wide = arm == "halo4w"
+        wp = _w_upfold_packed(weight_cl, 160 if wide else 80)
+        part = torch.empty(n, 4 * L.fmc_conv3x3_halo4_row_blocks_per_image(hs, ws), 32, 2, dtype=torch.float32, device=x_nhwc.device) if emit_gn else None
+        conv_halo_calls["conv4"] = conv_halo_calls.get("conv4", 0) + 1
+        if call_log is not None:
+            call_log.append(("conv_halo4", shape, flops))
+        _lib.check(L.fmc_conv3x3_halo4_fold_bf16(x_nhwc.data_ptr(), wp.data_ptr(), _p(bias), out.data_ptr(), n, hs, ws, cin, cout, _p(part), int(wide),
+                                                 _stream()), "fmc_conv3x3_halo4_fold_bf16")
+    return (out, part) if emit_gn else out
+
+
 F32_GEMM = os.environ.get("FMC_F32_GEMM", "1") != "0"
 f32_gemm_calls = {"linear": 0, "geglu": 0, "conv3x3": 0}
 
@@ -2252,6 +2348,20 @@
     stride2 = tuple(stride) == (2, 2)
     if stride2:
         h, w = h // 2, w // 2
+    if upsample and temb is None and r is None and not torch.is_grad_enabled() and x.dtype == torch.bfloat16 and weight_cl.dtype == torch.bfloat16:
+        arm = conv3x3_upfold_arm(n, h // 2, w // 2, cin, cout)
+        if arm is not None:
+            bn = 80 if arm == "halo4" else 160
+            want = bool(emit_gn and GN_EPILOGUE and cout % 64 == 0 and bn % (cout // 32) == 0 and (arm == "halo" or h * w >= GN_MIN_HW))
+            dispatch_calls["conv3x3"]["own"] += 1
+            y = conv3x3_upfold(x, weight_cl, bias, emit_gn=want, arm=arm)
+            if want:
+                y, part = y
+                gn_epilogue_calls["emitted"] += 1
+                y = y.permute(0, 3, 1, 2)
+                y._fmc_gn = (part, cout)
+                return y
+            return y.permute(0, 3, 1, 2)
     if (CONV_HALO and not stride2 and (temb is None or temb.stride(1) == 1) and conv3x3_halo_supported(n, h, w, cin, cin, cout, upsample)
             and n * _lib.load().fmc_conv3x3_halo_tiles_per_image(h, w) * (cout // 160) >= CONV_HALO_MIN_TILES):
         want = bool(emit_gn and GN_EPILOGUE and cout % 64 == 0 and 160 % (cout // 32) == 0 and not torch.is_grad_enabled())
```

After: 38.91 steps/s, median of 6. +1.1%, better.
